# MarcioCerqueira/RealTimeDepthDiffusion

Measured on AMD Instinct MI355X. Metric: Mpixel-iterations/s (solver sweep), higher is better.
Workload: dtype f32

## Files before the change

realtimedepthdiffusion_amd/csrc/api.cpp:

```cpp
#include <climits>
#include <cmath>
#include <cstring>
#include <new>

#include "rtdd_internal.hpp"
#include "persist_sync.hpp"

namespace rtdd {

int fail(rtdd_ctx *ctx, int status, const char *what, hipError_t e) {
    if (ctx) {
        ctx->last_error = what ? what : "";
        if (e != hipSuccess) {
            ctx->last_error += ": ";
            ctx->last_error += hipGetErrorString(e);
        }
    }
    return status;
}

void omega_schedule(int n, std::vector<float> &out) {
    out.resize(n > 0 ? n : 0);
    const int S = 10;
    float omega = 0.0f;
    const float rho = 0.99;
    for (int it = 0; it < n; it++) {
        if (it < S) omega = 1;
        else if (it == S) omega = 2.0 / (2.0 - rho * rho);
        else omega = 4.0 / (4.0 - rho * rho * omega);
        out[it] = omega;
    }
}

static void free_levels(rtdd_ctx *ctx) {
    for (auto &L : ctx->levels) {
        for (auto &p : L.plane)
            if (p) { (void)hipFree(p); p = nullptr; }
        if (L.meta) { (void)hipFree(L.meta); L.meta = nullptr; }
    }
    ctx->levels.clear();
    ctx->maxLevel = -1;
}

}

using namespace rtdd;

#pragma GCC visibility push(default)
extern "C" {

int rtdd_version(void) { return RTDD_VERSION; }

const char *rtdd_status_string(int s) {
    switch (s) {
        case RTDD_OK: return "ok";
        case RTDD_ERR_INVALID: return "invalid argument";
        case RTDD_ERR_STATE: return "call order violated";
        case RTDD_ERR_HIP: return "HIP runtime error";
        case RTDD_ERR_NOMEM: return "out of memory";
        case RTDD_ERR_NO_DEVICE: return "no usable HIP device (there is no CPU fallback)";
        case RTDD_ERR_TIMEOUT: return "persistent kernel timed out (workgroups not co-resident)";
        default: return "unknown status";
    }
}

const char *rtdd_last_error(rtdd_ctx *ctx) { return ctx ? ctx->last_error.c_str() : "null context"; }

int rtdd_ctx_create(int device, rtdd_ctx **out) {
    if (!out) return RTDD_ERR_INVALID;
    *out = nullptr;
    int n = 0;
    if (hipGetDeviceCount(&n) != hipSuccess || n <= 0) return RTDD_ERR_NO_DEVICE;
    if (device < 0 || device >= n) return RTDD_ERR_INVALID;
    rtdd_ctx *ctx = new (std::nothrow) rtdd_ctx();
    if (!ctx) return RTDD_ERR_NOMEM;
    ctx->device = device;
    for (auto &t : ctx->persist_fit) t[0] = t[1] = -1;
    DeviceGuard g(device);
    hipDeviceProp_t prop;
    if (hipGetDeviceProperties(&prop, device) == hipSuccess) ctx->num_cus = prop.multiProcessorCount > 0 ? prop.multiProcessorCount : 256;
    bool ok = hipMalloc((void **)&ctx->lut_dev, 257 * sizeof(float)) == hipSuccess &&
              hipMalloc((void **)&ctx->residual_dev, 64) == hipSuccess &&
              hipMalloc((void **)&ctx->sync_words, kSyncWords * sizeof(int)) == hipSuccess &&
              hipMemset(ctx->sync_words, 0, kSyncWords * sizeof(int)) == hipSuccess;
    for (auto &e : ctx->ev) ok = ok && hipEventCreate(&e) == hipSuccess;
    if (ok && hipHostMalloc((void **)&ctx->confirm_host, 64, hipHostMallocMapped) == hipSuccess) {
        *ctx->confirm_host = 0;
        void *dev_view = nullptr;
        ok = hipHostGetDevicePointer(&dev_view, ctx->confirm_host, 0) == hipSuccess &&
             hipMemcpy(ctx->sync_words + kSyncConfirmPtr, &dev_view, sizeof(dev_view), hipMemcpyHostToDevice) == hipSuccess;
    } else ok = false;
    if (!ok) { rtdd_ctx_destroy(ctx); return RTDD_ERR_HIP; }
    *out = ctx;
    return RTDD_OK;
}

int rtdd_ctx_destroy(rtdd_ctx *ctx) {
    if (!ctx) return RTDD_OK;
    DeviceGuard g(ctx->device);
    (void)hipStreamSynchronize(ctx->stream);
    pyramid_free(ctx);
    mg_release(ctx);
    free_levels(ctx);
    if (ctx->lut_dev) (void)hipFree(ctx->lut_dev);
    if (ctx->omega_dev) (void)hipFree(ctx->omega_dev);
    if (ctx->residual_dev) (void)hipFree(ctx->residual_dev);
    if (ctx->sync_words) (void)hipFree(ctx->sync_words);
    if (ctx->sat) (void)hipFree(ctx->sat);
    if (ctx->bounce.ptr) (void)hipFree(ctx->bounce.ptr);
    if (ctx->confirm_host) (void)hipHostFree(ctx->confirm_host);
    for (auto &e : ctx->ev) if (e) (void)hipEventDestroy(e);
    delete ctx;
    return RTDD_OK;
}

int rtdd_ctx_set_stream(rtdd_ctx *ctx, rtdd_stream stream) {
    if (!ctx) return RTDD_ERR_INVALID;
    DeviceGuard g(ctx->device);
    RTDD_TRY(settle_pending(ctx));
    ctx->stream = (hipStream_t)stream;
    return RTDD_OK;
}

int rtdd_ctx_synchronize(rtdd_ctx *ctx) {
    if (!ctx) return RTDD_ERR_INVALID;
    DeviceGuard g(ctx->device);
    RTDD_HIP(ctx, hipStreamSynchronize(ctx->stream));
    return check_persistent_status(ctx);
}

static const struct OptionRow {
    int key;
    int Options::*member;
    bool zero_or_one;
    int lo, hi; const char *refusal;
} kOptions[] = {
    {RTDD_OPT_FP_CONTRACT, &Options::fp_contract, true, 0, 1, nullptr},
    {RTDD_OPT_SWEEP_KERNEL, &Options::sweep_kernel, false, 0, 2, "sweep kernel must be 0..2"},
    {RTDD_OPT_TEMPORAL_DEPTH, &Options::temporal_depth, false, 0, 28, "temporal depth must be 0..28"},
    {RTDD_OPT_ROWS_PER_WAVE, &Options::rows_per_wave, false, 0, 1024, "rows per wave must be 0..1024"},
    {RTDD_OPT_DEFOCUS_PATH, &Options::defocus_path, false, 0, 2, "defocus path must be 0..2"},
    {RTDD_OPT_TILE, &Options::tile, false, 0, 16, "tile must be 0..16"},
    {RTDD_OPT_PERSISTENT, &Options::persistent, true, 0, 1, nullptr},
    {RTDD_OPT_ANNOTATION_LDS, &Options::annotation_lds, true, 0, 1, nullptr},
    {RTDD_OPT_LIVE_ZERO_COPY, &Options::live_zero_copy, false, 0, 2, "RTDD_OPT_LIVE_ZERO_COPY is 0, 1 or 2"},
    {RTDD_OPT_TIMEOUT_HEAL, &Options::timeout_heal, true, 0, 1, nullptr},
    {RTDD_OPT_PERSISTENT_REARM_AFTER, &Options::rearm_after, false, 0, 1 << 20, "must be 0..2^20"},
    {RTDD_OPT_DEFOCUS_SLICE_MB, &Options::defocus_slice_mb, false, 0, 4095, "must be 0..4095 MB"},
    {RTDD_OPT_DEFOCUS_STRIPS, &Options::defocus_strips, false, 0, 2, "must be 0, 1 or 2"},
    {RTDD_OPT_AUTO_CYCLE_FIXED_NS, &Options::auto_cycle_fixed_ns, false, 0, INT_MAX, "must be >= 0"},
    {RTDD_OPT_AUTO_CYCLE_FS_PER_PX, &Options::auto_cycle_fs_per_px, false, 0, INT_MAX, "must be >= 0"},
    {RTDD_OPT_AUTO_SWEEP_FS_PER_PX, &Options::auto_sweep_fs_per_px, false, 0, INT_MAX, "must be >= 0"},
    {RTDD_OPT_AUTO_SWEEP_FLOOR_NS, &Options::auto_sweep_floor_ns, false, 0, INT_MAX, "must be >= 0"},
    {RTDD_OPT_DEBUG_WITHHOLD_TILE, &Options::debug_withhold_tile, false, 0, kSyncMaxTiles, "tile number + 1 out of range"},
    {RTDD_OPT_DEBUG_POLL_LIMIT_US, &Options::debug_poll_limit_us, false, 0, 10000000, "poll limit must be 0..1e7 us"},
    {RTDD_OPT_DEBUG_FORCE_STATUS, &Options::debug_force_status, false, 0, 3, "status must be 0..3"},
};
static const OptionRow *find_option(int key) {
    for (const OptionRow &r : kOptions) if (r.key == key) return &r;
    return nullptr;
}

int rtdd_set_option(rtdd_ctx *ctx, int key, int value) {
    if (!ctx) return RTDD_ERR_INVALID;
    const OptionRow *r = find_option(key);
    if (!r) return fail(ctx, RTDD_ERR_INVALID, "unknown option");
    if (r->zero_or_one) value = value ? 1 : 0;
    else REQUIRE(ctx, value >= r->lo && value <= r->hi, r->refusal);
    ctx->opt.*(r->member) = value;
    switch (key) {
        case RTDD_OPT_DEFOCUS_PATH: if (value == 0) ctx->defocus_table_sticky = ctx->defocus_band_sticky = false; break;
        case RTDD_OPT_PERSISTENT: ctx->persistent_wanted = value; ctx->persist_suspend = 0; break;
        case RTDD_OPT_TIMEOUT_HEAL: if (!value && !ctx->healing) { ctx->pending.clear(); ctx->pending_overflow = false; } break;
        default: break;
    }
    return RTDD_OK;
}

int rtdd_get_option(rtdd_ctx *ctx, int key, int *value) {
    if (!ctx || !value) return RTDD_ERR_INVALID;
    if (const OptionRow *r = find_option(key)) { *value = ctx->opt.*(r->member); return RTDD_OK; }
    switch (key) {
        case RTDD_OPT_TIMEOUT_HEALS: *value = ctx->heals; break;
        case RTDD_OPT_DEFOCUS_LAST_PATH: *value = ctx->defocus_last_path; break;
        case RTDD_OPT_DEFOCUS_LAST_SLICES: *value = ctx->defocus_last_slices; break;
        case RTDD_OPT_PERSISTENT_SUSPENDED: *value = ctx->persist_suspend; break;
        case RTDD_OPT_PENDING_CALLS: prune_confirmed(ctx); *value = (int)ctx->pending.size(); break;
        default: return fail(ctx, RTDD_ERR_INVALID, "unknown option");
    }
    return RTDD_OK;
}

int rtdd_profile_enable(rtdd_ctx *ctx, int on) {
    if (!ctx) return RTDD_ERR_INVALID;
    ctx->profile_on = on != 0;
    ctx->prof_pending = 0;
    return RTDD_OK;
}

int rtdd_profile_get(rtdd_ctx *ctx, rtdd_profile *out) {
    if (!ctx || !out) return RTDD_ERR_INVALID;
    DeviceGuard g(ctx->device);
    rtdd_profile p{};
    const int n = ctx->prof_pending < rtdd_ctx::kProfSlots ? ctx->prof_pending : rtdd_ctx::kProfSlots;
    for (int i = 0; i < n; i++) {
        const int slot = (ctx->prof_pending - 1 - i) % rtdd_ctx::kProfSlots;
        hipEvent_t *ev = ctx->ev + 4 * slot;
        RTDD_HIP(ctx, hipEventSynchronize(ev[3]));
        float a = 0, b = 0, c = 0;
        RTDD_HIP(ctx, hipEventElapsedTime(&a, ev[0], ev[1]));
        RTDD_HIP(ctx, hipEventElapsedTime(&b, ev[1], ev[2]));
        RTDD_HIP(ctx, hipEventElapsedTime(&c, ev[2], ev[3]));
        p.prepare_ms += a; p.sweep_ms += b; p.finish_ms += c;
        p.launches += ctx->prof_launches[slot]; p.sweeps += ctx->prof_sweeps[slot];
    }
    ctx->prof_pending = 0;
    ctx->prof = p;
    *out = p;
    return RTDD_OK;
}


int rtdd_allocate(rtdd_ctx *ctx, int rows, int cols, int levels) {
    if (!ctx) return RTDD_ERR_INVALID;
    REQUIRE(ctx, rows > 0 && cols > 0 && levels > 0 && levels <= 30, "rows, cols, levels must be positive");
    DeviceGuard g(ctx->device);
    RTDD_TRY(settle_pending(ctx));
    RTDD_HIP(ctx, hipStreamSynchronize(ctx->stream));
    free_levels(ctx);
    const int images = ctx->alloc_images > 0 ? ctx->alloc_images : 1;
    ctx->alloc_images = 1;
    ctx->levels.resize(levels);
    for (int l = 0; l < levels; l++) {
        Level &L = ctx->levels[l];
        L.rows = (int)(rows / powf(2, l));
        L.cols = (int)(cols / powf(2, l));
        L.elems = plane_elems(L.rows > 0 ? L.rows : 1, L.cols > 0 ? L.cols : 1);
        const size_t all = L.elems * (size_t)images;
        for (auto &p : L.plane) {
            hipError_t e = hipMalloc((void **)&p, all * sizeof(float));
            if (e != hipSuccess) { free_levels(ctx); return fail(ctx, e == hipErrorOutOfMemory ? RTDD_ERR_NOMEM : RTDD_ERR_HIP,
                "hipMalloc(plane)", e); }
        }
        hipError_t e = hipMalloc((void **)&L.meta, all * sizeof(uint32_t));
        if (e != hipSuccess) { free_levels(ctx); return fail(ctx, e == hipErrorOutOfMemory ? RTDD_ERR_NOMEM : RTDD_ERR_HIP,
            "hipMalloc(meta)", e); }
        for (auto &p : L.plane) RTDD_HIP(ctx, hipMemsetAsync(p, 0, all * sizeof(float), ctx->stream));
        RTDD_HIP(ctx, hipMemsetAsync(L.meta, 0, all * sizeof(uint32_t), ctx->stream));
    }
    ctx->levels_images = images;
    ctx->maxLevel = levels - 1;
    RTDD_HIP(ctx, hipStreamSynchronize(ctx->stream));
    return RTDD_OK;
}

int rtdd_free(rtdd_ctx *ctx) {
    if (!ctx) return RTDD_ERR_INVALID;
    DeviceGuard g(ctx->device);
    RTDD_TRY(settle_pending(ctx));
    RTDD_HIP(ctx, hipStreamSynchronize(ctx->stream));
    mg_release(ctx);
    free_levels(ctx);
    return RTDD_OK;
}

int rtdd_load_weights(rtdd_ctx *ctx, float beta) {
    if (!ctx) return RTDD_ERR_INVALID;
    DeviceGuard g(ctx->device);
    RTDD_TRY(settle_pending(ctx));
    for (int w = 0; w < 256; w++) ctx->lut_host[w] = expf(-beta * w);
    ctx->lut_host[256] = 0;
    RTDD_HIP(ctx, hipMemcpyAsync(ctx->lut_dev, ctx->lut_host, sizeof(ctx->lut_host), hipMemcpyHostToDevice, ctx->stream));
    RTDD_HIP(ctx, hipStreamSynchronize(ctx->stream));
    ctx->weights_loaded = true;
    return RTDD_OK;
}

static int ensure_omegas(rtdd_ctx *ctx, int n) {
    if (n <= ctx->omega_cap) return RTDD_OK;
    int cap = n < 1024 ? 1024 : n;
    std::vector<float> om;
    omega_schedule(cap, om);
    RTDD_HIP(ctx, hipStreamSynchronize(ctx->stream));
    if (ctx->omega_dev) { RTDD_HIP(ctx, hipFree(ctx->omega_dev)); ctx->omega_dev = nullptr; ctx->omega_cap = 0; }
    RTDD_HIP(ctx, hipMalloc((void **)&ctx->omega_dev, (size_t)cap * sizeof(float)));
    RTDD_HIP(ctx, hipMemcpy(ctx->omega_dev, om.data(), (size_t)cap * sizeof(float), hipMemcpyHostToDevice));
    ctx->omega_cap = cap;
    return RTDD_OK;
}

static constexpr int kAutoMaxCycles = 60;

static int check_solve_args(rtdd_ctx *ctx, const SolveCall &c) {
    REQUIRE(ctx, c.depth && c.scribble && c.gray, "null image pointer");
    REQUIRE(ctx, c.rows > 0 && c.cols > 0, "rows and cols must be positive");
    REQUIRE(ctx, f32_image_aligned(c.depth, c.depthPitch), kF32AlignText);
    REQUIRE(ctx, c.depthPitch >= (size_t)c.cols * sizeof(float), "depth pitch smaller than a row");
    REQUIRE(ctx, c.guide == RTDD_GUIDE_GRAY || c.guide == RTDD_GUIDE_BGR, "unknown guide kind");
    REQUIRE(ctx, c.scribblePitch >= (size_t)c.cols && c.grayPitch >= (size_t)c.cols * (c.guide == RTDD_GUIDE_BGR ? 3 : 1), "u8 pitch smaller than a row");
    REQUIRE(ctx, (c.regionFlags & ~(RTDD_REGION_CUT | RTDD_REGION_SMOOTH)) == 0, "unknown region flag");
    REQUIRE(ctx, c.regionFlags == 0 || (c.regions && c.regionsPitch >= (size_t)c.cols), "region flags without a region image, or its pitch smaller than a row");
    if (ctx->levels.empty()) return fail(ctx, RTDD_ERR_STATE, "rtdd_allocate has not been called");
    if (!ctx->weights_loaded) return fail(ctx, RTDD_ERR_STATE, "rtdd_load_weights has not been called");
    REQUIRE(ctx, c.level >= 0 && c.level < (int)ctx->levels.size(), "level out of range");
    const Level &L = ctx->levels[c.level];
    REQUIRE(ctx, plane_elems(c.rows, c.cols) <= L.elems, "rows x cols exceeds the level's allocation");
    return RTDD_OK;
}

namespace {

struct Solve {
    rtdd_ctx *ctx;
    const Level &L;
    size_t ip;
    int rows, cols;
    const rtdd_solve_params *p;
    int images;
    int done = 0, launches = 0, cycles = 0;
    int pk = 0, pm = 1;
    float residual = NAN;

    bool stop_on_residual() const { return p->tolerance > 0.0f; }
    bool reached() const { return residual <= p->tolerance; }
    int check() { return launch_residual(ctx, L, ip, pk, rows, cols, &residual); }

    int chebyshev_jacobi() {
        std::vector<float> omegas;
        omega_schedule(p->maxIterations, omegas);
        const bool blocked = ctx->opt.sweep_kernel != 1;
        const float *omegas_dev = nullptr;
        int rc;
        if (blocked && p->maxIterations > 0) {
            if ((rc = ensure_omegas(ctx, p->maxIterations)) != RTDD_OK) return rc;
            omegas_dev = ctx->omega_dev;
        }
        const int chunk = stop_on_residual() ? (p->checkEvery > 0 ? p->checkEvery : 16) : p->maxIterations;
        while (done < p->maxIterations) {
            const int n = p->maxIterations - done < chunk ? p->maxIterations - done : chunk;
            int ln = 0;
            rc = blocked ? launch_sweeps_blocked(ctx, L, ip, rows, cols, omegas_dev + done, n, &pk, &pm, &ln, images)
                         : launch_sweeps(ctx, L, ip, rows, cols, omegas.data() + done, n, &pk, &pm, &ln);
            if (rc != RTDD_OK) return rc;
            done += n; launches += ln;
            if (stop_on_residual()) {
                if ((rc = check()) != RTDD_OK) return rc;
                if (reached()) break;
            }
        }
        return RTDD_OK;
    }

    int red_black_sweeps(int n, float omega) {
        if (n > p->maxIterations - done) n = p->maxIterations - done;
        if (n <= 0) return RTDD_OK;
        int ln = 2 * n, rc;
        if (ctx->opt.sweep_kernel == 1) rc = launch_rbgs(ctx, L, ip, pk, rows, cols, n, omega);
        else rc = launch_rbgs_blocked(ctx, L, ip, rows, cols, n, omega, &pk, &ln);
        done += n; launches += ln;
        return rc;
    }

    int red_black() {
        const int chunk = stop_on_residual() ? (p->checkEvery > 0 ? p->checkEvery : 16) : (p->maxIterations > 0 ? p->maxIterations : 1);
        const float omega = p->relaxation == 0.0f ? 1.0f : p->relaxation;
        int rc;
        while (done < p->maxIterations) {
            if ((rc = red_black_sweeps(chunk, omega)) != RTDD_OK) return rc;
            if (stop_on_residual()) {
                if ((rc = check()) != RTDD_OK) return rc;
                if (reached()) break;
            }
        }
        return RTDD_OK;
    }

    int sor_cycles(bool after_vcycles) {
        const int longest = rows > cols ? rows : cols;
        const int base = after_vcycles ? (longest + 1) / 2 : longest;
        double w0 = 2.0 / (1.0 + sin(4.0 * 3.14159265358979323846 / (double)longest));
        if (w0 > 1.99) w0 = 1.99;
        if (w0 < 1.0) w0 = 1.0;
        bool ok = false;
        int rc;
        for (int cycle = 0; done < p->maxIterations && !ok; cycle++) {
            const int e = cycle < 6 ? cycle : 6;
            double gap = (2.0 - w0) / (double)(1 << e);
            if (gap < 0.005) gap = 0.005;
            const float w_hi = (float)(2.0 - gap);
            float w_mid = (float)(2.0 - 10.0 * gap);
            if (w_mid < 1.0f) w_mid = 1.0f;
            const int n_hi = base << e;
            if ((rc = red_black_sweeps(n_hi, w_hi)) != RTDD_OK) return rc;
            if ((rc = red_black_sweeps(n_hi / 4, w_mid)) != RTDD_OK) return rc;
            for (int k = 0; k < 5 && done < p->maxIterations && !ok; k++) {
                if ((rc = red_black_sweeps(20, 1.0f)) != RTDD_OK) return rc;
                if (stop_on_residual()) {
                    if ((rc = check()) != RTDD_OK) return rc;
                    ok = reached();
                }
            }
        }
        return RTDD_OK;
    }

    int vcycles(int max_cycles, int check_every, double alternative_seconds) {
        const double px = (double)rows * cols;
        const double cycle_seconds = ctx->opt.auto_cycle_fixed_ns * 1e-9 + px * ctx->opt.auto_cycle_fs_per_px * 1e-15;
        return launch_multigrid(ctx, L, ip, rows, cols, max_cycles, p->tolerance, check_every, alternative_seconds, cycle_seconds, &pk,
            &cycles, &residual, &launches);
    }

    int automatic() {
        const int longest = rows > cols ? rows : cols;
        const double px = (double)rows * cols;
        const double per_px = px * ctx->opt.auto_sweep_fs_per_px * 1e-15, floor_s = ctx->opt.auto_sweep_floor_ns * 1e-9;
        const double sweep_seconds = per_px > floor_s ? per_px : floor_s;
        const double sor_seconds = ((double)((longest + 1) / 2) * 1.25 + 20.0) * sweep_seconds;
        const int rc = vcycles(kAutoMaxCycles, 1, sor_seconds);
        if (rc != RTDD_OK || reached()) return rc;
        return sor_cycles(true);
    }
};

}

static int solve_once(rtdd_ctx *ctx, const SolveCall &c, int seq, SolveOutcome *out) {
    const SolveTargets &t = c.targets;
    const Level L = ctx->levels[c.level].view(t.batch.first);
    const size_t ip = plane_pitch(c.cols);
    const bool prof = ctx->profile_on;
    hipEvent_t *ev = ctx->ev + 4 * (ctx->prof_pending % rtdd_ctx::kProfSlots);

    if (prof) RTDD_HIP(ctx, hipEventRecord(ev[0], ctx->stream));
    ctx->wild_seq = seq;
    int rc = launch_prepare(ctx, L, ip, c);
    if (rc != RTDD_OK) return rc;
    if (prof) RTDD_HIP(ctx, hipEventRecord(ev[1], ctx->stream));

    ctx->last_info = rtdd_solve_info{};
    ctx->last_info.residual = NAN;
    Solve s{ctx, L, ip, c.rows, c.cols, &c.params, t.batch.n};
    switch (c.params.method) {
        case RTDD_METHOD_CHEBYSHEV_JACOBI: rc = s.chebyshev_jacobi(); break;
        case RTDD_METHOD_MULTIGRID:
            rc = s.vcycles(c.params.maxIterations, c.params.checkEvery > 0 ? c.params.checkEvery : 1, 0.0);
            s.done = s.cycles;
            break;
        case RTDD_METHOD_AUTO: rc = s.automatic(); break;
        default: rc = c.params.relaxation < 0.0f ? s.sor_cycles(false) : s.red_black(); break;
    }
    if (rc != RTDD_OK) return rc;

    if (prof) RTDD_HIP(ctx, hipEventRecord(ev[2], ctx->stream));
    if (out) { out->plane = s.pk; out->seq = seq; }
    if (!t.defer_finish) {
        rc = launch_finish(ctx, L, ip, s.pk, c, seq);
        if (rc != RTDD_OK) return rc;
    }
    if (prof) {
        RTDD_HIP(ctx, hipEventRecord(ev[3], ctx->stream));
        const int slot = ctx->prof_pending % rtdd_ctx::kProfSlots;
        ctx->prof_launches[slot] = s.launches; ctx->prof_sweeps[slot] = s.done;
        ctx->prof_pending++;
    }
    ctx->last_info.iterations = s.done; ctx->last_info.residual = s.residual; ctx->last_info.cycles = s.cycles;
    ctx->last_info.fp_contract = ctx->opt.fp_contract; ctx->last_info.launches = s.launches;
    return RTDD_OK;
}

int rtdd_solve_ex(rtdd_ctx *ctx, float *depth, size_t depthPitch, const uint8_t *scribble, size_t scribblePitch,
                  const uint8_t *gray, size_t grayPitch, int rows, int cols, int level,
                  const rtdd_solve_params *params, rtdd_solve_info *info) {
    if (!ctx) return RTDD_ERR_INVALID;
    REQUIRE(ctx, params != nullptr, "null params");
    return solve_with(ctx, {depth, depthPitch, scribble, scribblePitch, gray, grayPitch, RTDD_GUIDE_GRAY, rows, cols, level, *params, {}}, info, nullptr);
}

int rtdd_solve_guided(rtdd_ctx *ctx, float *depth, size_t depthPitch, const uint8_t *scribble, size_t scribblePitch,
                      const uint8_t *guide, size_t guidePitch, int guideKind, int rows, int cols, int level,
                      const rtdd_solve_params *params, rtdd_solve_info *info) {
    if (!ctx) return RTDD_ERR_INVALID;
    REQUIRE(ctx, params != nullptr, "null params");
    return solve_with(ctx, {depth, depthPitch, scribble, scribblePitch, guide, guidePitch, guideKind, rows, cols, level, *params, {}}, info, nullptr);
}

int rtdd_solve_regions(rtdd_ctx *ctx, float *depth, size_t depthPitch, const uint8_t *scribble, size_t scribblePitch,
                       const uint8_t *guide, size_t guidePitch, int guideKind, const uint8_t *regions, size_t regionsPitch, int regionFlags,
                       int rows, int cols, int level, const rtdd_solve_params *params, rtdd_solve_info *info) {
    if (!ctx) return RTDD_ERR_INVALID;
    REQUIRE(ctx, params != nullptr, "null params");
    REQUIRE(ctx, (regionFlags & ~(RTDD_REGION_CUT | RTDD_REGION_SMOOTH)) == 0, "unknown region flag");
    REQUIRE(ctx, regions || regionFlags == 0, "region flags without a region image");
    REQUIRE(ctx, !regions || cols <= 0 || regionsPitch >= (size_t)cols, "region pitch smaller than a row");
    SolveCall c{depth, depthPitch, scribble, scribblePitch, guide, guidePitch, guideKind, rows, cols, level, *params, {}};
    if (regions && regionFlags != 0) { c.regions = regions; c.regionsPitch = regionsPitch; c.regionFlags = regionFlags; }
    return solve_with(ctx, c, info, nullptr);
}

}
#pragma GCC visibility pop

int rtdd::solve_with(rtdd_ctx *ctx, const SolveCall &c, rtdd_solve_info *info, SolveOutcome *out) {
    if (!ctx) return RTDD_ERR_INVALID;
    const SolveTargets &t = c.targets;
    REQUIRE(ctx, c.params.maxIterations >= 0, "maxIterations must be >= 0");
    REQUIRE(ctx, c.params.method == RTDD_METHOD_CHEBYSHEV_JACOBI || c.params.method == RTDD_METHOD_RED_BLACK_GS ||
                 c.params.method == RTDD_METHOD_MULTIGRID || c.params.method == RTDD_METHOD_AUTO, "unknown method");
    REQUIRE(ctx, c.params.method != RTDD_METHOD_AUTO || c.params.tolerance > 0.0f, "RTDD_METHOD_AUTO needs a tolerance");
    REQUIRE(ctx, c.params.method != RTDD_METHOD_RED_BLACK_GS || c.params.relaxation == RTDD_RELAXATION_AUTO ||
                 (c.params.relaxation >= 0.0f && c.params.relaxation < 2.0f), "relaxation must be in [0,2) or RTDD_RELAXATION_AUTO");
    RTDD_TRY(check_solve_args(ctx, c));
    REQUIRE(ctx, t.batch.first >= 0 && t.batch.n >= 1 && t.batch.first + t.batch.n <= ctx->levels_images,
            "the batch exceeds what the context's levels were allocated for");
    REQUIRE(ctx, t.batch.n == 1 || (c.params.method == RTDD_METHOD_CHEBYSHEV_JACOBI && c.params.tolerance <= 0.0f && ctx->opt.sweep_kernel != 1),
            "a batched solve runs the reference's scheme with the temporally blocked kernel only");
    DeviceGuard g(ctx->device);
    if (ctx->solve_seq >= (1 << 30)) {
        if (!ctx->healing) RTDD_TRY(settle_pending(ctx));
        RTDD_HIP(ctx, hipStreamSynchronize(ctx->stream));
        *(volatile int *)ctx->confirm_host = 0;
        RTDD_HIP(ctx, hipMemset(ctx->sync_words + kSyncWild, 0, sizeof(int)));
        ctx->solve_seq = 0; ctx->publish_seq = 0;
    }
    const int seq = ++ctx->solve_seq;
    const Options asked = ctx->opt;
    int rc = solve_once(ctx, c, seq, out);
    if (rc == kRestartSolve) rc = solve_once(ctx, c, seq, out);
    if (rc == kRestartSolve) rc = fail(ctx, RTDD_ERR_TIMEOUT, "the solve was restarted after a timed-out persistent launch and failed again");
    if (rc != RTDD_OK) return rc;
    if (!ctx->healing && ctx->persist_suspend > 0 && --ctx->persist_suspend == 0 && ctx->persistent_wanted) ctx->opt.persistent = 1;
    if (t.logged) {
        PendingOp op;
        op.kind = PendingOp::kSolve; op.opt = asked; op.solve = c; op.seq = seq;
        log_call(ctx, op);
    }
    if (info) *info = ctx->last_info;
    return RTDD_OK;
}

#pragma GCC visibility push(default)
extern "C" {

int rtdd_last_solve_info(rtdd_ctx *ctx, rtdd_solve_info *info) {
    if (!ctx || !info) return RTDD_ERR_INVALID;
    *info = ctx->last_info;
    return RTDD_OK;
}

int rtdd_multigrid_level(rtdd_ctx *ctx, int level, int which, float *host, int *rows, int *cols) {
    if (!ctx) return RTDD_ERR_INVALID;
    REQUIRE(ctx, rows && cols, "null size pointers");
    DeviceGuard g(ctx->device);
    const int rc = mg_download(ctx, level, which, host, rows, cols);
    if (rc == RTDD_ERR_INVALID) return fail(ctx, rc, "no multigrid hierarchy, or level/plane out of range");
    return rc;
}

int rtdd_matrix_free_solver(rtdd_ctx *ctx, float *depth, size_t depthPitch, const uint8_t *scribble, size_t scribblePitch,
                            const uint8_t *gray, size_t grayPitch, int rows, int cols, float beta, int maxIterations,
                            float tolerance, int level) {
    (void)beta; (void)tolerance;
    if (!ctx) return RTDD_ERR_INVALID;
    if (maxIterations < 0) maxIterations = 0;
    const rtdd_solve_params p{RTDD_METHOD_CHEBYSHEV_JACOBI, maxIterations, 0.0f, 0, 0.0f};
    return solve_with(ctx, {depth, depthPitch, scribble, scribblePitch, gray, grayPitch, RTDD_GUIDE_GRAY, rows, cols, level, p, {}}, nullptr, nullptr);
}

int rtdd_index_to_weight(rtdd_ctx *ctx, const uint8_t *gray, size_t grayPitch, const float *depth, size_t depthPitch,
                         int32_t *index2, int level, int rows, int cols) {
    return rtdd_index_to_weight_guided(ctx, gray, grayPitch, RTDD_GUIDE_GRAY, depth, depthPitch, index2, level, rows, cols);
}

int rtdd_index_to_weight_guided(rtdd_ctx *ctx, const uint8_t *guide, size_t guidePitch, int guideKind, const float *depth, size_t depthPitch,
                                int32_t *index2, int level, int rows, int cols) {
    return rtdd_index_to_weight_regions(ctx, guide, guidePitch, guideKind, nullptr, 0, 0, depth, depthPitch, index2, level, rows, cols);
}

int rtdd_index_to_weight_regions(rtdd_ctx *ctx, const uint8_t *guide, size_t guidePitch, int guideKind, const uint8_t *regions, size_t regionsPitch,
                                 int regionFlags, const float *depth, size_t depthPitch, int32_t *index2, int level, int rows, int cols) {
    if (!ctx) return RTDD_ERR_INVALID;
    REQUIRE(ctx, (regionFlags & ~(RTDD_REGION_CUT | RTDD_REGION_SMOOTH)) == 0, "unknown region flag");
    REQUIRE(ctx, regions || regionFlags == 0, "region flags without a region image");
    REQUIRE(ctx, !regions || cols <= 0 || regionsPitch >= (size_t)cols, "region pitch smaller than a row");
    if (!regions) regionFlags = 0;
    const uint8_t *gray = guide;
    REQUIRE(ctx, guideKind == RTDD_GUIDE_GRAY || guideKind == RTDD_GUIDE_BGR, "unknown guide kind");
    const size_t grayPitch = guideKind == RTDD_GUIDE_BGR ? guidePitch / 3 : guidePitch;
    REQUIRE(ctx, gray && depth && index2, "null pointer");
    REQUIRE(ctx, rows > 0 && cols > 0 && grayPitch >= (size_t)cols && depthPitch >= (size_t)cols * 4, "bad size or pitch");
    REQUIRE(ctx, f32_image_aligned(depth, depthPitch), kF32AlignText);
    if (ctx->maxLevel < 0) return fail(ctx, RTDD_ERR_STATE, "rtdd_allocate has not been called (maxLevel unknown)");
    DeviceGuard g(ctx->device);
    RTDD_TRY(settle_pending(ctx));
    return launch_index_to_weight(ctx, guide, guidePitch, depth, depthPitch, index2, level, rows, cols, guideKind, regions, regionsPitch, regionFlags);
}

int rtdd_region_codes(rtdd_ctx *ctx, const uint8_t *edited, size_t editedPitch, const uint8_t *mask, size_t maskPitch, int rows, int cols,
                      int level, uint8_t *codes, size_t codesPitch) {
    if (!ctx) return RTDD_ERR_INVALID;
    REQUIRE(ctx, edited && mask && codes, "null image pointer");
    REQUIRE(ctx, rows >= 0 && cols >= 0 && rows <= 32768 && cols <= 32768, "size outside [0, 32768]");
    REQUIRE(ctx, level >= 0 && level < 16, "level outside [0, 15]");
    RegionLevels lv{};
    lv.n = 1; lv.shift[0] = level; lv.rows[0] = rows >> level; lv.cols[0] = cols >> level;
    if (lv.rows[0] == 0 || lv.cols[0] == 0) return RTDD_OK;
    REQUIRE(ctx, editedPitch >= (size_t)cols * 3 && maskPitch >= (size_t)cols && codesPitch >= (size_t)lv.cols[0], "pitch smaller than a row");
    lv.codes[0] = codes; lv.pitch[0] = codesPitch; lv.stride[0] = 0;
    DeviceGuard g(ctx->device);
    RTDD_TRY(pyramid_check_read(ctx, mask, edited));
    return launch_region_codes(ctx, edited, editedPitch, 0, mask, maskPitch, 0, lv, 1);
}

}
#pragma GCC visibility pop
```

realtimedepthdiffusion_amd/csrc/rtdd_internal.hpp:

```cpp
#pragma once

#include <hip/hip_runtime.h>

#include <cmath>
#include <cstdint>
#include <cstdio>
#include <string>
#include <vector>

#include "rtdd.h"

namespace rtdd {

constexpr int kGuardRows = 16;
constexpr int kGuardCols = 64;
constexpr int kRowAlign = 64;

inline size_t plane_pitch(int cols) { return (size_t)((cols + kRowAlign - 1) / kRowAlign) * kRowAlign + kGuardCols; }
inline size_t plane_elems(int rows, int cols) { return plane_pitch(cols) * (size_t)(rows + 2 * kGuardRows) + 1024; }

constexpr uint32_t kMetaDirichlet = 1u << 16;

struct Level {
    int rows = 0, cols = 0;
    size_t elems = 0;
    float *plane[4] = {nullptr, nullptr, nullptr, nullptr};
    uint32_t *meta = nullptr;
    float *P(int i, size_t ip) const { return plane[i] + (size_t)kGuardRows * ip; }
    uint32_t *M(size_t ip) const { return meta + (size_t)kGuardRows * ip; }
    Level view(int b) const {
        Level v = *this;
        for (auto &q : v.plane) if (q) q += (size_t)b * elems;
        if (v.meta) v.meta += (size_t)b * elems;
        return v;
    }
};

struct Batch {
    int n = 1;
    int first = 0;
    size_t depth = 0, scribble = 0, gray = 0, u8 = 0;
    size_t regions = 0;
};
#define RTDD_Z(ptr, stride) ptr = (decltype(ptr))((const char *)(ptr) + (size_t)blockIdx.z * (size_t)(stride))

struct SolveTargets {
    Batch batch;
    bool defer_finish = false;
    uint8_t *u8 = nullptr; size_t u8_pitch = 0;
    uint8_t *u8b = nullptr; size_t u8b_pitch = 0;
    bool logged = true;
};
struct SolveOutcome { int seq = 0, plane = -1; };
struct SolveCall {
    float *depth = nullptr; size_t depthPitch = 0;
    const uint8_t *scribble = nullptr; size_t scribblePitch = 0;
    const uint8_t *gray = nullptr; size_t grayPitch = 0;
    int guide = RTDD_GUIDE_GRAY;
    int rows = 0, cols = 0, level = 0;
    rtdd_solve_params params{};
    SolveTargets targets;
    const uint8_t *regions = nullptr; size_t regionsPitch = 0;
    int regionFlags = 0;
};
struct LiveTargets {
    void *scribble = nullptr, *edited = nullptr;
    uint8_t *u8 = nullptr; size_t u8_pitch = 0;
    int effect = 0;
    uint8_t *artistic = nullptr; size_t artistic_pitch = 0;
};

struct Effect {
    enum : int { kRefocus = RTDD_EFFECT_HAZE + 1, kHazeEx, kStereo, kLensBlur, kRelight, kRelightShadow, kParallax, kAmbientOcclusion, kLighting, kBokeh, kComposite, kRemove, kLift, kParallaxLayered };
    int kind = RTDD_EFFECT_NONE;
    const uint8_t *original = nullptr; size_t originalPitch = 0;
    const float *depth = nullptr; size_t depthPitch = 0;
    uint8_t *artistic = nullptr; size_t artisticPitch = 0;
    int rows = 0, cols = 0;
    const uint8_t *gray = nullptr; size_t grayPitch = 0;
    int kernelSize = 0, focusX = -1, focusY = -1;
    float focusDepth = 0.0f;
    float beta = 2.0f; uint32_t air = 0xFFFFFFu;
    int disparity = 0, zeroX = -1, zeroY = -1, stereoMode = 0;
    float zeroDepth = 0.0f;
    struct Light {
        int kind = 0, anchorX = -1, anchorY = -1;
        float x = 0.0f, y = 0.0f, z = 1.0f;
        float anchorDepth = 0.0f, invR2 = 0.0f;
        float relief = 0.0f, ambient = 0.0f, k[3] = {0.0f, 0.0f, 0.0f};
    } light = {};
    struct Shadow {
        float sx = 0.0f, sy = 0.0f, rise = 0.0f;
        int maxSteps = 0;
        float bias = 0.0f, softness = 0.0f, strength = 0.0f;
    } shadow = {};
    struct Parallax {
        int shiftX = 0, shiftY = 0, zeroX = -1, zeroY = -1;
        float dolly = 0.0f, zeroDepth = 0.0f;
        float cx = 0.0f, cy = 0.0f;
    } parallax = {};
    struct ParallaxLayers {
        const uint8_t *plate = nullptr; size_t platePitch = 0;
        const float *plateDepth = nullptr; size_t plateDepthPitch = 0;
        float *depthOut = nullptr; size_t depthOutPitch = 0;
        uint8_t *coverage = nullptr; size_t coveragePitch = 0;
    } layers = {};
    struct Occlusion {
        int mode = 0, directions = 8, radius = 0;
        float relief = 0.0f, bias = 0.0f, strength = 0.0f;
        bool lit = false;
    } occlusion = {};
    struct Composite {
        rtdd_layer layer = {};
        const uint8_t *sprite = nullptr; size_t spritePitch = 0;
        float *depthOut = nullptr; size_t depthOutPitch = 0;
        int fx0 = 0, fy0 = 0, fx1 = 0, fy1 = 0;
    } composite = {};
    struct Remove {
        rtdd_removal removal = {};
        const uint8_t *mask = nullptr; size_t maskPitch = 0;
        float *depthOut = nullptr; size_t depthOutPitch = 0;
    } remove = {};
    struct Lift {
        const uint8_t *mask = nullptr; size_t maskPitch = 0;
        int select = 0, x = 0, y = 0;
        uint8_t *sprite = nullptr; size_t spritePitch = 0;
        int spriteRows = 0, spriteCols = 0;
    } lift = {};
};

inline int window_scale(double aperture, int rows, int cols) {
    const double k = aperture * sqrtf(rows * rows + cols * cols);
    return k < 2147483647.0 ? (int)k : 2147483647;
}

struct Options {
    int fp_contract = 1;
    int sweep_kernel = 0;
    int temporal_depth = 0;
    int rows_per_wave = 0;
    int tile = 0;
    int persistent = 1;
    int defocus_path = 0;
    int auto_cycle_fixed_ns = 270000;
    int auto_cycle_fs_per_px = 46000;
    int auto_sweep_fs_per_px = 1429;
    int auto_sweep_floor_ns = 2500;
    int debug_withhold_tile = 0;
    int debug_poll_limit_us = 0;
    int debug_force_status = 0;
    int timeout_heal = 1;
    int annotation_lds = 1;
    int live_zero_copy = 1;
    int defocus_slice_mb = 0;
    int defocus_strips = 0;
    int rearm_after = 64;
};

struct PendingOp {
    enum Kind { kSolve = 0, kEstimate = 1, kEffect = 2 } kind = kSolve;
    Options opt;
    unsigned long long id = 0;
    SolveCall solve;
    int seq = 0;
    struct Estimate {
        int maxIterations = 0;
        int level_seq[32] = {};
        int batch_first = 0, batch_n = 1;
        int guide = RTDD_GUIDE_GRAY;
        int regionFlags = 0;
        LiveTargets live;
        int annotation = 0;
    } estimate;
    enum : int { kAnnotationNone = 0, kAnnotationAccumulated = 1, kAnnotationRebuilt = 2 };
    Effect effect;
};
constexpr int kRestartSolve = -1000;
constexpr size_t kMaxPendingOps = 4096;
constexpr int kMaxRearms = 4;

}

namespace rtdd { struct Pyramid; struct MgState; }

namespace rtdd {
struct Bounce { void *ptr = nullptr; size_t bytes = 0; };
}

struct rtdd_ctx {
    int device = 0;
    rtdd::Pyramid *pyr = nullptr;
    rtdd::MgState *mg = nullptr;
    hipStream_t stream = nullptr;
    std::vector<rtdd::Level> levels;
    int alloc_images = 1;
    int levels_images = 1;
    int maxLevel = -1;
    bool weights_loaded = false;
    float lut_host[257];
    float *lut_dev = nullptr;
    float *omega_dev = nullptr;
    int omega_cap = 0;
    float *residual_dev = nullptr;
    int *sync_words = nullptr;
    int defocus_last_path = 0;
    int defocus_last_slices = 0;
    bool defocus_band_sticky = false;
    bool defocus_table_sticky = false;
    int flag_epoch = 0;
    int sync_limit = 0;
    int last_nominal_depth = 0;
    int last_launch_images = 1;
    rtdd_solve_info last_info{};
    int solve_seq = 0;
    int wild_seq = -1;
    std::vector<rtdd::PendingOp> pending;
    bool pending_overflow = false;
    bool healing = false;
    bool heal_rebuilt = false;
    bool heal_warned = false;
    int heals = 0;
    int persistent_wanted = 1;
    int persist_suspend = 0;
    int *confirm_host = nullptr;
    unsigned long long op_counter = 0;
    bool persistent_used = false;
    int publish_seq = 0;
    bool status_writer_behind = false;
    signed char persist_fit[17][2];
    rtdd::Bounce bounce;
    uint32_t *sat = nullptr;
    size_t sat_elems = 0;
    int sat_rows = 0, sat_cols = 0;
    int num_cus = 256;
    rtdd::Options opt;
    bool profile_on = false;
    rtdd_profile prof{};
    static constexpr int kProfSlots = 64;
    hipEvent_t ev[4 * kProfSlots] = {};
    int prof_launches[kProfSlots] = {}, prof_sweeps[kProfSlots] = {};
    int prof_pending = 0;
    std::string last_error;
};

namespace rtdd {

#ifdef __HIPCC__
__device__ __forceinline__ int wave_id() { return __builtin_amdgcn_readfirstlane((int)(threadIdx.x >> 6)); }
#endif

int fail(rtdd_ctx *ctx, int status, const char *what, hipError_t e = hipSuccess);
inline bool f32_image_aligned(const void *p, size_t pitch) { return (uintptr_t)p % sizeof(float) == 0 && pitch % sizeof(float) == 0; }
constexpr const char *kF32AlignText = "an f32 image needs a pointer and a pitch that are multiples of 4";
inline void note_status_writer(rtdd_ctx *ctx) { ctx->persistent_used = true; ctx->status_writer_behind = true; }
inline void note_publisher(rtdd_ctx *ctx, int seq) { ctx->persistent_used = true; ctx->publish_seq = seq; ctx->status_writer_behind = false; }

#define RTDD_HIP(ctx, call)                                                        \
    do {                                                                           \
        hipError_t e_ = (call);                                                    \
        if (e_ != hipSuccess) return ::rtdd::fail((ctx), RTDD_ERR_HIP, #call, e_); \
    } while (0)

#define REQUIRE(ctx, cond, msg) \
    do { if (!(cond)) return ::rtdd::fail((ctx), RTDD_ERR_INVALID, msg); } while (0)
#define REQUIRE_PYRAMID(ctx)                                                                                             \
    do {                                                                                                                 \
        if (!(ctx)) return RTDD_ERR_INVALID;                                                                             \
        if (!(ctx)->pyr) return ::rtdd::fail((ctx), RTDD_ERR_STATE, "rtdd_pyramid_create has not been called");          \
    } while (0)
#define RTDD_TRY(call) \
    do { const int rc_ = (call); if (rc_ != RTDD_OK) return rc_; } while (0)

#define RTDD_LAUNCH_CHECK(ctx, name)                                                     \
    do {                                                                                 \
        hipError_t e_ = hipGetLastError();                                               \
        if (e_ != hipSuccess) return ::rtdd::fail((ctx), RTDD_ERR_HIP, "launch " name, e_); \
    } while (0)

struct DeviceGuard {
    int prev = -1;
    explicit DeviceGuard(int dev) {
        if (hipGetDevice(&prev) != hipSuccess) prev = -1;
        if (prev != dev) (void)hipSetDevice(dev);
        else prev = -1;
    }
    ~DeviceGuard() {
        if (prev >= 0) (void)hipSetDevice(prev);
    }
};

int launch_prepare(rtdd_ctx *ctx, const Level &L, size_t ip, const SolveCall &c);
int launch_sweeps(rtdd_ctx *ctx, const Level &L, size_t ip, int rows, int cols, const float *omegas_host, int n,
                  int *pk, int *pm, int *launches);
int launch_sweeps_blocked(rtdd_ctx *ctx, const Level &L, size_t ip, int rows, int cols, const float *omegas_dev, int n,
                          int *pk, int *pm, int *launches, int images = 1);
int launch_finish(rtdd_ctx *ctx, const Level &L, size_t ip, int src_plane, const SolveCall &c, int seq);
int launch_index_to_weight(rtdd_ctx *ctx, const uint8_t *gray, size_t grayPitch, const float *depth, size_t depthPitch,
                           int32_t *index2, int level, int rows, int cols, int guide = RTDD_GUIDE_GRAY,
                           const uint8_t *regions = nullptr, size_t regionsPitch = 0, int regionFlags = 0);
int launch_residual(rtdd_ctx *ctx, const Level &L, size_t ip, int plane, int rows, int cols, float *host_out);
int launch_rbgs(rtdd_ctx *ctx, const Level &L, size_t ip, int plane, int rows, int cols, int nsweeps, float omega);
int launch_multigrid(rtdd_ctx *ctx, const Level &L0, size_t ip, int rows, int cols, int max_cycles, float tolerance, int check_every, double alternative_seconds,
                     double cycle_seconds, int *plane, int *cycles_done, float *residual, int *launches);
void mg_release(rtdd_ctx *ctx);
int mg_download(rtdd_ctx *ctx, int level, int which, float *host, int *rows, int *cols);

int launch_rbgs_blocked(rtdd_ctx *ctx, const Level &L, size_t ip, int rows, int cols, int n, float omega, int *plane, int *launches, int keep = -1);

int launch_convert(rtdd_ctx *ctx, const uint8_t *src, size_t srcPitch, float *dst, size_t dstPitch,
                   const uint8_t *mask, size_t maskPitch, int rows, int cols, int images = 1, size_t zSrc = 0, size_t zDst = 0, size_t zMask = 0);
int launch_pyrdown_annotation(rtdd_ctx *ctx, const uint8_t *ps, size_t psp, const uint8_t *pe, size_t pep, int prows, int pcols,
                              uint8_t *cs, size_t csp, uint8_t *ce, size_t cep, int crows, int ccols,
                              int images = 1, size_t zPs = 0, size_t zPe = 0, size_t zCs = 0, size_t zCe = 0);
int launch_annotation_pyramid(rtdd_ctx *ctx, int levels, uint8_t *const *scribble, const size_t *sp, const size_t *zs, uint8_t *const *edited, const size_t *ep, const size_t *ze,
                              const int *rows, const int *cols, float *depth, size_t dp, size_t zd, int images, bool rebuild = false);
int launch_repitch(rtdd_ctx *ctx, hipStream_t stream, const void *src, size_t srcPitch, void *dst, size_t dstPitch, size_t widthBytes, int rows);
inline bool slow_pitch(size_t hostPitch, int rows) { return hostPitch % 4 != 0 && rows > 1; }
inline bool wants_bounce(size_t hostPitch, size_t widthBytes, int rows) { return slow_pitch(hostPitch, rows) && hostPitch == widthBytes; }
int copy_h2d_linear(rtdd_ctx *ctx, Bounce &b, void *dev, size_t devPitch, const void *host, size_t hostPitch, size_t widthBytes, int rows,
                    hipStream_t copyStream, hipStream_t kernelStream);
int copy_h2d_repitch(rtdd_ctx *ctx, const Bounce &b, void *dev, size_t devPitch, size_t hostPitch, size_t widthBytes, int rows, hipStream_t kernelStream);
int copy_h2d(rtdd_ctx *ctx, Bounce &b, void *dev, size_t devPitch, const void *host, size_t hostPitch, size_t widthBytes, int rows, hipStream_t stream);
int copy_d2h(rtdd_ctx *ctx, Bounce &b, void *host, size_t hostPitch, const void *dev, size_t devPitch, size_t widthBytes, int rows, hipStream_t stream);
struct PaintTarget {
    uint8_t *edited; size_t editedPitch;
    uint8_t *scribble; size_t scribblePitch;
    const uint8_t *original; size_t originalPitch;
    int rows, cols;
};
int launch_paint(rtdd_ctx *ctx, int x, int y, int color, int radius, const PaintTarget &t);
template <class Stroke> int launch_paint_strokes(rtdd_ctx *ctx, const Stroke *strokes, int count, const PaintTarget &t);

int launch_fill_polygon(rtdd_ctx *ctx, const int *xy, int n, const rtdd_fill &fill, const PaintTarget &t);

int launch_fill_similar(rtdd_ctx *ctx, const rtdd_wand &wand, const PaintTarget &t, rtdd_wand_info *info);
int launch_fill_surface(rtdd_ctx *ctx, const rtdd_surface_wand &wand, const PaintTarget &t, const float *depth, size_t depthPitch, rtdd_wand_info *info);

int launch_segment_surfaces(rtdd_ctx *ctx, const rtdd_segmentation &sg, const PaintTarget &t, const float *depth, size_t depthPitch, int32_t *labels,
                            size_t labelsPitch, rtdd_segment *segments, rtdd_segment_info *info);

int launch_effect(rtdd_ctx *ctx, const Effect &e);
int launch_lens_blur(rtdd_ctx *ctx, const Effect &e);
int launch_relight(rtdd_ctx *ctx, const Effect &e);
int launch_relight_shadow(rtdd_ctx *ctx, const Effect &e);
int launch_parallax(rtdd_ctx *ctx, const Effect &e);
int launch_ambient_occlusion(rtdd_ctx *ctx, const Effect &e);
int launch_lighting(rtdd_ctx *ctx, const Effect &e);
int launch_bokeh(rtdd_ctx *ctx, const Effect &e);
int launch_composite(rtdd_ctx *ctx, const Effect &e);
constexpr int kRemoveTile = 64, kRemoveGroup = 3, kRemoveApex = 8192, kRemoveApexChain = kRemoveApex + kRemoveApex / 2 + 64;
int launch_remove(rtdd_ctx *ctx, const Effect &e);
int launch_lift(rtdd_ctx *ctx, const Effect &e);

int launch_bgr2gray(rtdd_ctx *ctx, const uint8_t *bgr, size_t bp, uint8_t *gray, size_t gp, int rows, int cols);
int launch_pyrdown_u8(rtdd_ctx *ctx, const uint8_t *src, size_t sp, int rows, int cols, uint8_t *dst, size_t dp);
int launch_pyrdown_bgr(rtdd_ctx *ctx, const uint8_t *src, size_t sp, int rows, int cols, uint8_t *dst, size_t dp);
struct PyrupBatch { int n = 1; size_t src = 0, dst = 0, edited = 0, mask = 0, coarse = 0; };
int launch_pyrup_inject(rtdd_ctx *ctx, const float *src, size_t sp, int rows, int cols, float *dst, size_t dp, int drows, int dcols,
                        const uint8_t *edited, size_t ep, const uint8_t *mask, size_t mp, float *coarse_out = nullptr, size_t cp = 0,
                        int guard_seq = 0 , const PyrupBatch *batch = nullptr);
int launch_depth_to_u8(rtdd_ctx *ctx, const float *src, size_t sp, uint8_t *dst, size_t dp, int rows, int cols);
int launch_decode_annotation(rtdd_ctx *ctx, const uint8_t *bgr, size_t bp, const uint8_t *ann, size_t ap, uint8_t *edited, size_t ep,
                             uint8_t *scribble, size_t sp, int rows, int cols);
int launch_fill_f32(rtdd_ctx *ctx, float *dst, size_t dp, int rows, int cols, float v);
struct RegionLevels {
    static constexpr int kMax = 12;
    int n = 0;
    uint8_t *codes[kMax]; size_t pitch[kMax], stride[kMax];
    int rows[kMax], cols[kMax], shift[kMax], first_block[kMax + 1];
};
int launch_region_codes(rtdd_ctx *ctx, const uint8_t *edited, size_t ep, size_t ze, const uint8_t *mask, size_t mp, size_t zm, RegionLevels &lv, int images);
void pyramid_free(rtdd_ctx *ctx);
int pyramid_note_write(rtdd_ctx *ctx, const void *scribble, const void *edited, bool erases = false);
int pyramid_check_read(rtdd_ctx *ctx, const void *a, const void *b);

int prepare_persistent_launch(rtdd_ctx *ctx, int nblocks, int *flag_base);
int check_persistent_status(rtdd_ctx *ctx, bool in_solve = false);
void prune_confirmed(rtdd_ctx *ctx);
int settle_pending(rtdd_ctx *ctx);
bool log_call(rtdd_ctx *ctx, PendingOp &op);
int solve_with(rtdd_ctx *ctx, const SolveCall &c, rtdd_solve_info *info, SolveOutcome *out);
int estimate_replay(rtdd_ctx *ctx, const PendingOp::Estimate &e, int failed_seq);

void omega_schedule(int n, std::vector<float> &out);

}
```

realtimedepthdiffusion_amd/csrc/solver_kernels.hip:

```cpp
#include "rtdd_internal.hpp"
#include "persist_sync.hpp"

namespace rtdd {

__device__ __forceinline__ int sat_u8_dev(float v) {
    if (!(v >= 0.0f)) return 0;
    if (v >= 255.0f) return 255;
    return (int)v;
}

__device__ __forceinline__ int iabs(int a) { return a < 0 ? -a : a; }

__device__ __forceinline__ int region_index(int i, int rp, int rq, int flags) {
    if ((flags & RTDD_REGION_CUT) && rp != rq) return 255;
    if ((flags & RTDD_REGION_SMOOTH) && rp == rq && rp != 0) return 0;
    return i;
}
#define RTDD_PREPARE_PARAMS(g, gp, zg)                                                                                                      \
    const float *__restrict__ depth, size_t depthPitch, const uint8_t *__restrict__ scribble, size_t scribblePitch,                         \
    const uint8_t *__restrict__ g, size_t gp, float *__restrict__ X0, float *__restrict__ X1, uint32_t *__restrict__ M, int ip, int rows,    \
    int cols, int gated, int thr, size_t zDepth, size_t zScribble, size_t zg, size_t zPlane, int *sync_words, int wild_seq
#define RTDD_PREPARE_ARGS(g, gp, zg) \
    depth, depthPitch, scribble, scribblePitch, g, gp, X0, X1, M, ip, rows, cols, gated, thr, zDepth, zScribble, zg, zPlane, sync_words, wild_seq
#define RTDD_REGION_PARAMS const uint8_t *__restrict__ codes, size_t codesPitch, size_t zCodes, int regionFlags
#define RTDD_REGION_ARGS codes, codesPitch, zCodes, regionFlags
#define RTDD_NO_REGIONS nullptr, 0, 0, 0

template <bool REGIONS>
__device__ __forceinline__ void prepare_px(RTDD_PREPARE_PARAMS(gray, grayPitch, zGray), RTDD_REGION_PARAMS) {
    const int x = blockIdx.x * 64 + (threadIdx.x & 63);
    const int y = blockIdx.y * 4 + wave_id();
    if (x >= cols || y >= rows) return;
    RTDD_Z(depth, zDepth); RTDD_Z(scribble, zScribble); RTDD_Z(gray, zGray); RTDD_Z(X0, zPlane); RTDD_Z(X1, zPlane); RTDD_Z(M, zPlane);
    const float *drow = (const float *)((const char *)depth + (size_t)y * depthPitch);
    const uint8_t *grow = gray + (size_t)y * grayPitch;
    const float d = drow[x];
    const int g = grow[x];
    const bool dirichlet = scribble[(size_t)y * scribblePitch + x] == 255;
    const uint8_t *rrow = nullptr;
    if (REGIONS) { RTDD_Z(codes, zCodes); rrow = codes + (size_t)y * codesPitch; }
    int right = 0, down = 0;
    if (x + 1 < cols) {
        right = iabs(g - (int)grow[x + 1]);
        if (gated && !(iabs(sat_u8_dev(d) - sat_u8_dev(drow[x + 1])) > thr)) right = 0;
        if (REGIONS) right = region_index(right, rrow[x], rrow[x + 1], regionFlags);
    }
    if (y + 1 < rows) {
        down = iabs(g - (int)grow[x + grayPitch]);
        if (gated) {
            const float dd = ((const float *)((const char *)depth + (size_t)(y + 1) * depthPitch))[x];
            if (!(iabs(sat_u8_dev(d) - sat_u8_dev(dd)) > thr)) down = 0;
        }
        if (REGIONS) down = region_index(down, rrow[x], rrow[x + codesPitch], regionFlags);
    }
    const size_t p = (size_t)y * ip + x;
    if (depth_is_wild(d)) sync_words[kSyncWild] = wild_seq;
    X0[p] = d;
    X1[p] = dirichlet ? d : 0.0f;
    M[p] = (uint32_t)right | ((uint32_t)down << 8) | (dirichlet ? kMetaDirichlet : 0u);
}
__global__ __launch_bounds__(256) void k_prepare(RTDD_PREPARE_PARAMS(gray, grayPitch, zGray)) {
    prepare_px<false>(RTDD_PREPARE_ARGS(gray, grayPitch, zGray), RTDD_NO_REGIONS);
}
__global__ __launch_bounds__(256) void k_prepare_regions(RTDD_PREPARE_PARAMS(gray, grayPitch, zGray), RTDD_REGION_PARAMS) {
    prepare_px<true>(RTDD_PREPARE_ARGS(gray, grayPitch, zGray), RTDD_REGION_ARGS);
}

struct RegionCodes4 { int rc[5], rd[4]; };
template <bool REGIONS>
__device__ __forceinline__ void load_codes4(RegionCodes4 &r, const uint8_t *rrow, size_t codesPitch, int x0, int cols, bool down_ok) {
    if (!REGIONS) return;
    if (x0 + 3 < cols) {
        const uint32_t c4 = *(const uint32_t *)(rrow + x0);
        r.rc[0] = c4 & 255; r.rc[1] = (c4 >> 8) & 255; r.rc[2] = (c4 >> 16) & 255; r.rc[3] = c4 >> 24;
        if (down_ok) {
            const uint32_t e4 = *(const uint32_t *)(rrow + codesPitch + x0);
            r.rd[0] = e4 & 255; r.rd[1] = (e4 >> 8) & 255; r.rd[2] = (e4 >> 16) & 255; r.rd[3] = e4 >> 24;
        }
    } else {
#pragma unroll
        for (int i = 0; i < 4; i++) {
            const bool in = x0 + i < cols;
            r.rc[i] = in ? rrow[x0 + i] : 0;
            r.rd[i] = in && down_ok ? rrow[x0 + i + codesPitch] : 0;
        }
    }
    r.rc[4] = x0 + 4 < cols ? rrow[x0 + 4] : 0;
}

template <bool REGIONS>
__device__ __forceinline__ void prepare4_px(RTDD_PREPARE_PARAMS(gray, grayPitch, zGray), RTDD_REGION_PARAMS) {
    const int x0 = 4 * (blockIdx.x * 64 + (threadIdx.x & 63));
    const int y = blockIdx.y * 4 + wave_id();
    if (x0 >= cols || y >= rows) return;
    RTDD_Z(depth, zDepth); RTDD_Z(scribble, zScribble); RTDD_Z(gray, zGray); RTDD_Z(X0, zPlane); RTDD_Z(X1, zPlane); RTDD_Z(M, zPlane);
    const float *drow = (const float *)((const char *)depth + (size_t)y * depthPitch);
    const uint8_t *grow = gray + (size_t)y * grayPitch, *srow = scribble + (size_t)y * scribblePitch;
    const bool down_ok = y + 1 < rows;
    float d[5], dd[4];
    int g[5], gd[4];
    uint32_t sc;
    RegionCodes4 rg;
    if (REGIONS) { RTDD_Z(codes, zCodes); load_codes4<REGIONS>(rg, codes + (size_t)y * codesPitch, codesPitch, x0, cols, down_ok); }
    if (x0 + 3 < cols) {
        const float4 d4 = *(const float4 *)(drow + x0);
        d[0] = d4.x; d[1] = d4.y; d[2] = d4.z; d[3] = d4.w;
        const uint32_t g4 = *(const uint32_t *)(grow + x0);
        g[0] = g4 & 255; g[1] = (g4 >> 8) & 255; g[2] = (g4 >> 16) & 255; g[3] = g4 >> 24;
        sc = *(const uint32_t *)(srow + x0);
        if (down_ok) {
            const uint32_t h4 = *(const uint32_t *)(grow + grayPitch + x0);
            gd[0] = h4 & 255; gd[1] = (h4 >> 8) & 255; gd[2] = (h4 >> 16) & 255; gd[3] = h4 >> 24;
            if (gated) { const float4 e4 = *(const float4 *)((const float *)((const char *)depth + (size_t)(y + 1) * depthPitch) + x0); dd[0] = e4.x; dd[1] = e4.y; dd[2] = e4.z; dd[3] = e4.w; }
        }
    } else {
        sc = 0;
#pragma unroll
        for (int i = 0; i < 4; i++) {
            const bool in = x0 + i < cols;
            d[i] = in ? drow[x0 + i] : 0.0f; g[i] = in ? grow[x0 + i] : 0;
            sc |= (uint32_t)(in ? srow[x0 + i] : 0) << (8 * i);
            gd[i] = in && down_ok ? grow[x0 + i + grayPitch] : 0;
            dd[i] = in && down_ok && gated ? ((const float *)((const char *)depth + (size_t)(y + 1) * depthPitch))[x0 + i] : 0.0f;
        }
    }
    const bool right_ok = x0 + 4 < cols;
    d[4] = right_ok ? drow[x0 + 4] : 0.0f; g[4] = right_ok ? grow[x0 + 4] : 0;
    float x0v[4], x1v[4];
    uint32_t mv[4];
#pragma unroll
    for (int i = 0; i < 4; i++) {
        const bool dirichlet = ((sc >> (8 * i)) & 255) == 255;
        int right = 0, down = 0;
        if (x0 + i + 1 < cols) {
            right = iabs(g[i] - g[i + 1]);
            if (gated && !(iabs(sat_u8_dev(d[i]) - sat_u8_dev(d[i + 1])) > thr)) right = 0;
            if (REGIONS) right = region_index(right, rg.rc[i], rg.rc[i + 1], regionFlags);
        }
        if (down_ok) {
            down = iabs(g[i] - gd[i]);
            if (gated && !(iabs(sat_u8_dev(d[i]) - sat_u8_dev(dd[i])) > thr)) down = 0;
            if (REGIONS) down = region_index(down, rg.rc[i], rg.rd[i], regionFlags);
        }
        x0v[i] = d[i];
        x1v[i] = dirichlet ? d[i] : 0.0f;
        mv[i] = (uint32_t)right | ((uint32_t)down << 8) | (dirichlet ? kMetaDirichlet : 0u);
    }
    if (depth_is_wild(d[0]) || depth_is_wild(d[1]) || depth_is_wild(d[2]) || depth_is_wild(d[3])) sync_words[kSyncWild] = wild_seq;
    const size_t p = (size_t)y * ip + x0;
    *(float4 *)(X0 + p) = make_float4(x0v[0], x0v[1], x0v[2], x0v[3]);
    *(float4 *)(X1 + p) = make_float4(x1v[0], x1v[1], x1v[2], x1v[3]);
    *(uint4 *)(M + p) = make_uint4(mv[0], mv[1], mv[2], mv[3]);
}
__global__ __launch_bounds__(256) void k_prepare4(RTDD_PREPARE_PARAMS(gray, grayPitch, zGray)) {
    prepare4_px<false>(RTDD_PREPARE_ARGS(gray, grayPitch, zGray), RTDD_NO_REGIONS);
}
__global__ __launch_bounds__(256) void k_prepare4_regions(RTDD_PREPARE_PARAMS(gray, grayPitch, zGray), RTDD_REGION_PARAMS) {
    prepare4_px<true>(RTDD_PREPARE_ARGS(gray, grayPitch, zGray), RTDD_REGION_ARGS);
}

template <bool REGIONS> struct RegionImage {};
template <> struct RegionImage<true> { const uint8_t *codes; size_t pitch; int flags; };
__device__ __forceinline__ int region_index(int i, int x, int y, int nx, int ny, const RegionImage<true> &rg) {
    return region_index(i, rg.codes[(size_t)y * rg.pitch + x], rg.codes[(size_t)ny * rg.pitch + nx], rg.flags);
}
__device__ __forceinline__ int region_index(int i, int, int, int, int, const RegionImage<false> &) { return i; }

template <bool REGIONS>
__global__ __launch_bounds__(256) void k_index_to_weight(const uint8_t *__restrict__ gray, size_t grayPitch,
                                                         const float *__restrict__ depth, size_t depthPitch,
                                                         int32_t *__restrict__ index2, int rows, int cols, int gated, int thr, const RegionImage<REGIONS> rg) {
    const int x = blockIdx.x * 64 + (threadIdx.x & 63);
    const int y = blockIdx.y * 4 + wave_id();
    if (x >= cols || y >= rows) return;
    const int g = gray[(size_t)y * grayPitch + x];
    const float *drow = (const float *)((const char *)depth + (size_t)y * depthPitch);
    const int d = gated ? sat_u8_dev(drow[x]) : 0;
    int idx[4] = {256, 256, 256, 256};
    const int dx[4] = {-1, 1, 0, 0}, dy[4] = {0, 0, -1, 1};
#pragma unroll
    for (int k = 0; k < 4; k++) {
        const int nx = x + dx[k], ny = y + dy[k];
        if (nx < 0 || ny < 0 || nx >= cols || ny >= rows) continue;
        int v = iabs(g - (int)gray[(size_t)ny * grayPitch + nx]);
        if (gated) {
            const float nd = ((const float *)((const char *)depth + (size_t)ny * depthPitch))[nx];
            if (!(iabs(d - sat_u8_dev(nd)) > thr)) v = 0;
        }
        if (REGIONS) v = region_index(v, x, y, nx, ny, rg);
        idx[k] = v;
    }
    const size_t p = (size_t)y * cols + x;
    index2[2 * p + 0] = idx[0] * 1000 + idx[1];
    index2[2 * p + 1] = idx[2] * 1000 + idx[3];
}

__device__ __forceinline__ int bgr_at(const uint8_t *p) { return (int)p[0] | ((int)p[1] << 8) | ((int)p[2] << 16); }
__device__ __forceinline__ int bgr_index(int p, int q) {
    const int db = iabs((p & 255) - (q & 255)), dg = iabs(((p >> 8) & 255) - ((q >> 8) & 255)), dr = iabs((p >> 16) - (q >> 16));
    return max(max(db, dg), dr);
}

template <bool REGIONS>
__device__ __forceinline__ void prepare_bgr_px(RTDD_PREPARE_PARAMS(bgr, bgrPitch, zBgr), RTDD_REGION_PARAMS) {
    const int x = blockIdx.x * 64 + (threadIdx.x & 63);
    const int y = blockIdx.y * 4 + wave_id();
    if (x >= cols || y >= rows) return;
    RTDD_Z(depth, zDepth); RTDD_Z(scribble, zScribble); RTDD_Z(bgr, zBgr); RTDD_Z(X0, zPlane); RTDD_Z(X1, zPlane); RTDD_Z(M, zPlane);
    const float *drow = (const float *)((const char *)depth + (size_t)y * depthPitch);
    const uint8_t *crow = bgr + (size_t)y * bgrPitch + 3 * (size_t)x;
    const float d = drow[x];
    const int c = bgr_at(crow);
    const bool dirichlet = scribble[(size_t)y * scribblePitch + x] == 255;
    const uint8_t *rrow = nullptr;
    if (REGIONS) { RTDD_Z(codes, zCodes); rrow = codes + (size_t)y * codesPitch; }
    int right = 0, down = 0;
    if (x + 1 < cols) {
        right = bgr_index(c, bgr_at(crow + 3));
        if (gated && !(iabs(sat_u8_dev(d) - sat_u8_dev(drow[x + 1])) > thr)) right = 0;
        if (REGIONS) right = region_index(right, rrow[x], rrow[x + 1], regionFlags);
    }
    if (y + 1 < rows) {
        down = bgr_index(c, bgr_at(crow + bgrPitch));
        if (gated) {
            const float dd = ((const float *)((const char *)depth + (size_t)(y + 1) * depthPitch))[x];
            if (!(iabs(sat_u8_dev(d) - sat_u8_dev(dd)) > thr)) down = 0;
        }
        if (REGIONS) down = region_index(down, rrow[x], rrow[x + codesPitch], regionFlags);
    }
    const size_t p = (size_t)y * ip + x;
    if (depth_is_wild(d)) sync_words[kSyncWild] = wild_seq;
    X0[p] = d;
    X1[p] = dirichlet ? d : 0.0f;
    M[p] = (uint32_t)right | ((uint32_t)down << 8) | (dirichlet ? kMetaDirichlet : 0u);
}
__global__ __launch_bounds__(256) void k_prepare_bgr(RTDD_PREPARE_PARAMS(bgr, bgrPitch, zBgr)) {
    prepare_bgr_px<false>(RTDD_PREPARE_ARGS(bgr, bgrPitch, zBgr), RTDD_NO_REGIONS);
}
__global__ __launch_bounds__(256) void k_prepare_bgr_regions(RTDD_PREPARE_PARAMS(bgr, bgrPitch, zBgr), RTDD_REGION_PARAMS) {
    prepare_bgr_px<true>(RTDD_PREPARE_ARGS(bgr, bgrPitch, zBgr), RTDD_REGION_ARGS);
}

__device__ __forceinline__ void bgr_unpack4(const uint8_t *q, int (&c)[5]) {
    const uint32_t *w = (const uint32_t *)q;
    const uint32_t w0 = w[0], w1 = w[1], w2 = w[2];
    c[0] = (int)(w0 & 0xFFFFFFu); c[1] = (int)((w0 >> 24) | ((w1 & 0xFFFFu) << 8));
    c[2] = (int)((w1 >> 16) | ((w2 & 0xFFu) << 16)); c[3] = (int)(w2 >> 8);
}

template <bool REGIONS>
__device__ __forceinline__ void prepare4_bgr_px(RTDD_PREPARE_PARAMS(bgr, bgrPitch, zBgr), RTDD_REGION_PARAMS) {
    const int x0 = 4 * (blockIdx.x * 64 + (threadIdx.x & 63));
    const int y = blockIdx.y * 4 + wave_id();
    if (x0 >= cols || y >= rows) return;
    RTDD_Z(depth, zDepth); RTDD_Z(scribble, zScribble); RTDD_Z(bgr, zBgr); RTDD_Z(X0, zPlane); RTDD_Z(X1, zPlane); RTDD_Z(M, zPlane);
    const float *drow = (const float *)((const char *)depth + (size_t)y * depthPitch);
    const uint8_t *crow = bgr + (size_t)y * bgrPitch + 3 * (size_t)x0, *srow = scribble + (size_t)y * scribblePitch;
    const bool down_ok = y + 1 < rows;
    float d[5], dd[4];
    int c[5], cd[5];
    uint32_t sc;
    RegionCodes4 rg;
    if (REGIONS) { RTDD_Z(codes, zCodes); load_codes4<REGIONS>(rg, codes + (size_t)y * codesPitch, codesPitch, x0, cols, down_ok); }
    if (x0 + 3 < cols) {
        const float4 d4 = *(const float4 *)(drow + x0);
        d[0] = d4.x; d[1] = d4.y; d[2] = d4.z; d[3] = d4.w;
        bgr_unpack4(crow, c);
        sc = *(const uint32_t *)(srow + x0);
        if (down_ok) {
            bgr_unpack4(crow + bgrPitch, cd);
            if (gated) { const float4 e4 = *(const float4 *)((const float *)((const char *)depth + (size_t)(y + 1) * depthPitch) + x0); dd[0] = e4.x; dd[1] = e4.y; dd[2] = e4.z; dd[3] = e4.w; }
        }
    } else {
        sc = 0;
#pragma unroll
        for (int i = 0; i < 4; i++) {
            const bool in = x0 + i < cols;
            d[i] = in ? drow[x0 + i] : 0.0f; c[i] = in ? bgr_at(crow + 3 * i) : 0;
            sc |= (uint32_t)(in ? srow[x0 + i] : 0) << (8 * i);
            cd[i] = in && down_ok ? bgr_at(crow + bgrPitch + 3 * i) : 0;
            dd[i] = in && down_ok && gated ? ((const float *)((const char *)depth + (size_t)(y + 1) * depthPitch))[x0 + i] : 0.0f;
        }
    }
    const bool right_ok = x0 + 4 < cols;
    d[4] = right_ok ? drow[x0 + 4] : 0.0f;
    c[4] = right_ok ? (int)*(const uint16_t *)(crow + 12) | ((int)crow[14] << 16) : 0;
    float x0v[4], x1v[4];
    uint32_t mv[4];
#pragma unroll
    for (int i = 0; i < 4; i++) {
        const bool dirichlet = ((sc >> (8 * i)) & 255) == 255;
        int right = 0, down = 0;
        if (x0 + i + 1 < cols) {
            right = bgr_index(c[i], c[i + 1]);
            if (gated && !(iabs(sat_u8_dev(d[i]) - sat_u8_dev(d[i + 1])) > thr)) right = 0;
            if (REGIONS) right = region_index(right, rg.rc[i], rg.rc[i + 1], regionFlags);
        }
        if (down_ok) {
            down = bgr_index(c[i], cd[i]);
            if (gated && !(iabs(sat_u8_dev(d[i]) - sat_u8_dev(dd[i])) > thr)) down = 0;
            if (REGIONS) down = region_index(down, rg.rc[i], rg.rd[i], regionFlags);
        }
        x0v[i] = d[i];
        x1v[i] = dirichlet ? d[i] : 0.0f;
        mv[i] = (uint32_t)right | ((uint32_t)down << 8) | (dirichlet ? kMetaDirichlet : 0u);
    }
    if (depth_is_wild(d[0]) || depth_is_wild(d[1]) || depth_is_wild(d[2]) || depth_is_wild(d[3])) sync_words[kSyncWild] = wild_seq;
    const size_t p = (size_t)y * ip + x0;
    *(float4 *)(X0 + p) = make_float4(x0v[0], x0v[1], x0v[2], x0v[3]);
    *(float4 *)(X1 + p) = make_float4(x1v[0], x1v[1], x1v[2], x1v[3]);
    *(uint4 *)(M + p) = make_uint4(mv[0], mv[1], mv[2], mv[3]);
}
__global__ __launch_bounds__(256) void k_prepare4_bgr(RTDD_PREPARE_PARAMS(bgr, bgrPitch, zBgr)) {
    prepare4_bgr_px<false>(RTDD_PREPARE_ARGS(bgr, bgrPitch, zBgr), RTDD_NO_REGIONS);
}
__global__ __launch_bounds__(256) void k_prepare4_bgr_regions(RTDD_PREPARE_PARAMS(bgr, bgrPitch, zBgr), RTDD_REGION_PARAMS) {
    prepare4_bgr_px<true>(RTDD_PREPARE_ARGS(bgr, bgrPitch, zBgr), RTDD_REGION_ARGS);
}

template <bool REGIONS>
__global__ __launch_bounds__(256) void k_index_to_weight_bgr(const uint8_t *__restrict__ bgr, size_t bgrPitch,
                                                             const float *__restrict__ depth, size_t depthPitch,
                                                             int32_t *__restrict__ index2, int rows, int cols, int gated, int thr, const RegionImage<REGIONS> rg) {
    const int x = blockIdx.x * 64 + (threadIdx.x & 63);
    const int y = blockIdx.y * 4 + wave_id();
    if (x >= cols || y >= rows) return;
    const int c = bgr_at(bgr + (size_t)y * bgrPitch + 3 * (size_t)x);
    const float *drow = (const float *)((const char *)depth + (size_t)y * depthPitch);
    const int d = gated ? sat_u8_dev(drow[x]) : 0;
    int idx[4] = {256, 256, 256, 256};
    const int dx[4] = {-1, 1, 0, 0}, dy[4] = {0, 0, -1, 1};
#pragma unroll
    for (int k = 0; k < 4; k++) {
        const int nx = x + dx[k], ny = y + dy[k];
        if (nx < 0 || ny < 0 || nx >= cols || ny >= rows) continue;
        int v = bgr_index(c, bgr_at(bgr + (size_t)ny * bgrPitch + 3 * (size_t)nx));
        if (gated) {
            const float nd = ((const float *)((const char *)depth + (size_t)ny * depthPitch))[nx];
            if (!(iabs(d - sat_u8_dev(nd)) > thr)) v = 0;
        }
        if (REGIONS) v = region_index(v, x, y, nx, ny, rg);
        idx[k] = v;
    }
    const size_t p = (size_t)y * cols + x;
    index2[2 * p + 0] = idx[0] * 1000 + idx[1];
    index2[2 * p + 1] = idx[2] * 1000 + idx[3];
}

template <bool CONTRACT>
__device__ __forceinline__ float mean4(float xl, float xr, float xu, float xd, float wl, float wr, float wu, float wd,
                                       bool vl, bool vr, bool vu, bool vd) {
    float sum = 0.0f, cnt = 0.0f, s2;
    s2 = CONTRACT ? __builtin_fmaf(wl, xl, sum) : sum + wl * xl;  sum = vl ? s2 : sum;  cnt = vl ? cnt + wl : cnt;
    s2 = CONTRACT ? __builtin_fmaf(wr, xr, sum) : sum + wr * xr;  sum = vr ? s2 : sum;  cnt = vr ? cnt + wr : cnt;
    s2 = CONTRACT ? __builtin_fmaf(wu, xu, sum) : sum + wu * xu;  sum = vu ? s2 : sum;  cnt = vu ? cnt + wu : cnt;
    s2 = CONTRACT ? __builtin_fmaf(wd, xd, sum) : sum + wd * xd;  sum = vd ? s2 : sum;  cnt = vd ? cnt + wd : cnt;
    float r = sum / cnt;
    if (!(r >= 0.0f)) r = 0.0f;
    if (r > 255.0f) r = 255.0f;
    if (cnt == 0.0f) r = 0.0f;
    return r;
}

template <bool CONTRACT>
__device__ __forceinline__ float chebyshev(float r, float x, float prev, float omega, float gamma) {
    if (CONTRACT) return __builtin_fmaf(omega, __builtin_fmaf(gamma, r - x, x) - prev, prev);
    return (omega * (gamma * (r - x) + x - prev)) + prev;
}

template <bool CONTRACT>
__global__ __launch_bounds__(256) void k_sweep1(const float *__restrict__ X, float *__restrict__ Y,
                                                const uint32_t *__restrict__ M, const float *__restrict__ lut_g,
                                                int ip, int rows, int cols, int R, float omega, float gamma) {
    __shared__ float lut[257];
    for (int i = threadIdx.x; i < 257; i += 256) lut[i] = lut_g[i];
    __syncthreads();

    const int lane = threadIdx.x & 63;
    const int wave = wave_id();
    const int x0 = blockIdx.x * 256 + lane * 4;
    const int ybeg = (blockIdx.y * 4 + wave) * R;
    const int yend = min(ybeg + R, rows);
    if (ybeg >= rows) return;

    const bool lane_in = x0 < cols;
    const bool vl0 = x0 > 0;
    bool vr[4];
#pragma unroll
    for (int i = 0; i < 4; i++) vr[i] = x0 + i + 1 < cols;

    const float *xrow = X + (size_t)ybeg * ip + x0;
    float4 up = *(const float4 *)(xrow - ip);
    float4 cur = *(const float4 *)(xrow);
    float wu[4];
    {
        const uint4 mu = *(const uint4 *)(M + (size_t)(ybeg - 1) * ip + x0);
        wu[0] = lut[(mu.x >> 8) & 255]; wu[1] = lut[(mu.y >> 8) & 255];
        wu[2] = lut[(mu.z >> 8) & 255]; wu[3] = lut[(mu.w >> 8) & 255];
    }

    for (int y = ybeg; y < yend; y++) {
        const size_t rowoff = (size_t)y * ip + x0;
        const float4 dn = *(const float4 *)(X + rowoff + ip);
        const uint4 m = *(const uint4 *)(M + rowoff);
        const float4 pv = *(const float4 *)(Y + rowoff);

        float xl = __shfl_up(cur.w, 1);
        float xr = __shfl_down(cur.x, 1);
        uint32_t ml = __shfl_up(m.w, 1);
        if (lane == 0) { xl = X[rowoff - 1]; ml = M[rowoff - 1]; }
        if (lane == 63) xr = X[rowoff + 4];

        const float wr[4] = {lut[m.x & 255], lut[m.y & 255], lut[m.z & 255], lut[m.w & 255]};
        const float wd[4] = {lut[(m.x >> 8) & 255], lut[(m.y >> 8) & 255], lut[(m.z >> 8) & 255], lut[(m.w >> 8) & 255]};
        const float wl0 = lut[ml & 255];
        const bool vu = y > 0, vd = y + 1 < rows;

        const float xc[4] = {cur.x, cur.y, cur.z, cur.w};
        const float xu[4] = {up.x, up.y, up.z, up.w};
        const float xd[4] = {dn.x, dn.y, dn.z, dn.w};
        const float pp[4] = {pv.x, pv.y, pv.z, pv.w};
        const uint32_t mm[4] = {m.x, m.y, m.z, m.w};
        float o[4];
#pragma unroll
        for (int i = 0; i < 4; i++) {
            const float r = mean4<CONTRACT>(i == 0 ? xl : xc[i - 1], i == 3 ? xr : xc[i + 1], xu[i], xd[i],
                                            i == 0 ? wl0 : wr[i - 1], wr[i], wu[i], wd[i],
                                            i == 0 ? vl0 : true, vr[i], vu, vd);
            const float v = chebyshev<CONTRACT>(r, xc[i], pp[i], omega, gamma);
            o[i] = (mm[i] & kMetaDirichlet) ? xc[i] : v;
        }
        if (lane_in) *(float4 *)(Y + rowoff) = make_float4(o[0], o[1], o[2], o[3]);
        up = cur; cur = dn;
#pragma unroll
        for (int i = 0; i < 4; i++) wu[i] = wd[i];
    }
}

__device__ __forceinline__ uint8_t round_u8(float v) {
    const float r = __builtin_rintf(v);
    return !(r >= 0.0f) ? 0 : (r >= 255.0f ? 255 : (uint8_t)(int)r);
}

__global__ __launch_bounds__(256) void k_finish(const float *__restrict__ X, int ip, float *__restrict__ depth, size_t depthPitch,
                                                int rows, int cols, uint8_t *__restrict__ u8, size_t u8Pitch, int *sync_words, int seq,
                                                size_t zPlane, size_t zDepth, size_t zU8, uint8_t *__restrict__ u8b, size_t u8bPitch) {
    const int x = blockIdx.x * 64 + (threadIdx.x & 63);
    const int y = blockIdx.y * 4 + wave_id();
    if (solve_is_dead(sync_words, seq, (blockIdx.x | blockIdx.y | blockIdx.z | threadIdx.x) == 0)) return;
    if (x >= cols || y >= rows) return;
    RTDD_Z(X, zPlane); RTDD_Z(depth, zDepth); if (u8) RTDD_Z(u8, zU8);
    const float v = X[(size_t)y * ip + x];
    ((float *)((char *)depth + (size_t)y * depthPitch))[x] = v;
    if (u8) u8[(size_t)y * u8Pitch + x] = round_u8(v);
    if (u8b) u8b[(size_t)y * u8bPitch + x] = round_u8(v);
}

__global__ __launch_bounds__(256) void k_finish4(const float *__restrict__ X, int ip, float *__restrict__ depth, size_t depthPitch,
                                                 int rows, int cols, uint8_t *__restrict__ u8, size_t u8Pitch, int *sync_words, int seq,
                                                 size_t zPlane, size_t zDepth, size_t zU8, uint8_t *__restrict__ u8b, size_t u8bPitch) {
    const int x0 = 4 * (blockIdx.x * 64 + (threadIdx.x & 63));
    const int y = blockIdx.y * 4 + wave_id();
    if (solve_is_dead(sync_words, seq, (blockIdx.x | blockIdx.y | blockIdx.z | threadIdx.x) == 0)) return;
    if (x0 >= cols || y >= rows) return;
    RTDD_Z(X, zPlane); RTDD_Z(depth, zDepth); if (u8) RTDD_Z(u8, zU8);
    const float4 v = *(const float4 *)(X + (size_t)y * ip + x0);
    float *o = (float *)((char *)depth + (size_t)y * depthPitch) + x0;
    const float t[4] = {v.x, v.y, v.z, v.w};
    if (x0 + 3 < cols) *(float4 *)o = v;
    else { for (int i = 0; i < 4; i++) if (x0 + i < cols) o[i] = t[i]; }
    uint8_t *targets[2] = {u8, u8b};
    const size_t pitches[2] = {u8Pitch, u8bPitch};
#pragma unroll
    for (int k = 0; k < 2; k++) {
        if (!targets[k]) continue;
        uint8_t *q = targets[k] + (size_t)y * pitches[k] + x0;
        if (x0 + 3 < cols && pitches[k] % 4 == 0 && (uintptr_t)targets[k] % 4 == 0)
            *(uint32_t *)q = (uint32_t)round_u8(t[0]) | ((uint32_t)round_u8(t[1]) << 8) | ((uint32_t)round_u8(t[2]) << 16) | ((uint32_t)round_u8(t[3]) << 24);
        else { for (int i = 0; i < 4; i++) if (x0 + i < cols) q[i] = round_u8(t[i]); }
    }
}

template <bool CONTRACT>
__device__ __forceinline__ float mean_at(const float *__restrict__ X, const uint32_t *__restrict__ M, const float *lut,
                                         int ip, int rows, int cols, int x, int y, uint32_t m) {
    const size_t p = (size_t)y * ip + x;
    const bool vl = x > 0, vr = x + 1 < cols, vu = y > 0, vd = y + 1 < rows;
    const uint32_t ml = M[p - 1], mu = M[p - ip];
    return mean4<CONTRACT>(X[p - 1], X[p + 1], X[p - ip], X[p + ip],
                           lut[ml & 255], lut[m & 255], lut[(mu >> 8) & 255], lut[(m >> 8) & 255], vl, vr, vu, vd);
}

template <bool CONTRACT>
__global__ __launch_bounds__(256) void k_residual(const float *__restrict__ X, const uint32_t *__restrict__ M,
                                                  const float *__restrict__ lut_g, int ip, int rows, int cols,
                                                  unsigned int *__restrict__ out_bits) {
    __shared__ float lut[257];
    __shared__ float wmax[4];
    for (int i = threadIdx.x; i < 257; i += 256) lut[i] = lut_g[i];
    __syncthreads();
    const int x0 = 4 * (blockIdx.x * 64 + (threadIdx.x & 63));
    const int y = blockIdx.y * 4 + wave_id();
    float d = 0.0f;
    if (x0 < cols && y < rows) {
        const size_t p = (size_t)y * ip + x0;
        const float4 c4 = *(const float4 *)(X + p), u4 = *(const float4 *)(X + p - ip), d4 = *(const float4 *)(X + p + ip);
        const uint4 m4 = *(const uint4 *)(M + p), mu4 = *(const uint4 *)(M + p - ip);
        const float xc[4] = {c4.x, c4.y, c4.z, c4.w}, xu[4] = {u4.x, u4.y, u4.z, u4.w}, xd[4] = {d4.x, d4.y, d4.z, d4.w};
        const uint32_t mm[4] = {m4.x, m4.y, m4.z, m4.w}, mu[4] = {mu4.x, mu4.y, mu4.z, mu4.w};
        const float xl0 = X[p - 1], xr4 = X[p + 4];
        const uint32_t ml0 = M[p - 1];
        const bool vu = y > 0, vd = y + 1 < rows;
#pragma unroll
        for (int i = 0; i < 4; i++) {
            const int x = x0 + i;
            if (x < cols && !(mm[i] & kMetaDirichlet)) {
                const float r = mean4<CONTRACT>(i == 0 ? xl0 : xc[i - 1], i == 3 ? xr4 : xc[i + 1], xu[i], xd[i],
                                                lut[(i == 0 ? ml0 : mm[i - 1]) & 255], lut[mm[i] & 255], lut[(mu[i] >> 8) & 255], lut[(mm[i] >> 8) & 255],
                                                x > 0, x + 1 < cols, vu, vd);
                float e = fabsf(r - xc[i]);
                if (!(e >= 0.0f)) e = __builtin_inff();
                d = fmaxf(d, e);
            }
        }
    }
#pragma unroll
    for (int s = 32; s > 0; s >>= 1) d = fmaxf(d, __shfl_xor(d, s));
    if ((threadIdx.x & 63) == 0) wmax[threadIdx.x >> 6] = d;
    __syncthreads();
    if (threadIdx.x == 0) {
        d = fmaxf(fmaxf(wmax[0], wmax[1]), fmaxf(wmax[2], wmax[3]));
        const unsigned int bits = __float_as_uint(d);
        if (bits > __hip_atomic_load(out_bits, __ATOMIC_RELAXED, __HIP_MEMORY_SCOPE_AGENT)) atomicMax(out_bits, bits);
    }
}

template <bool CONTRACT>
__global__ __launch_bounds__(256) void k_rbgs_half(float *__restrict__ X, const uint32_t *__restrict__ M,
                                                   const float *__restrict__ lut_g, int ip, int rows, int cols, int colour, float omega) {
    __shared__ float lut[257];
    for (int i = threadIdx.x; i < 257; i += 256) lut[i] = lut_g[i];
    __syncthreads();
    const int y = blockIdx.y * 4 + wave_id();
    const int x = 2 * (blockIdx.x * 64 + (threadIdx.x & 63)) + ((y + colour) & 1);
    if (x >= cols || y >= rows) return;
    const uint32_t m = M[(size_t)y * ip + x];
    if (m & kMetaDirichlet) return;
    float v = mean_at<CONTRACT>(X, M, lut, ip, rows, cols, x, y, m);
    if (omega != 1.0f) {
        const float x0 = X[(size_t)y * ip + x];
        v = CONTRACT ? __builtin_fmaf(omega, v - x0, x0) : x0 + omega * (v - x0);
        v = fminf(fmaxf(v, 0.0f), 255.0f);
    }
    X[(size_t)y * ip + x] = v;
}

static inline dim3 grid64x4(int rows, int cols, int images = 1) { return dim3((cols + 63) / 64, (rows + 3) / 4, images); }

int launch_prepare(rtdd_ctx *ctx, const Level &L, size_t ip, const SolveCall &c) {
    const Batch &B = c.targets.batch;
    const int gated = c.level != ctx->maxLevel;
    const int thr = c.level == 0 ? 0 : 4;
    const size_t zP = L.elems * sizeof(float);
    bool aligned = ((uintptr_t)c.depth % 16 == 0) && c.depthPitch % 16 == 0 && ((uintptr_t)c.gray % 4 == 0) && c.grayPitch % 4 == 0 &&
                         ((uintptr_t)c.scribble % 4 == 0) && c.scribblePitch % 4 == 0 && B.depth % 16 == 0 && B.gray % 4 == 0 && B.scribble % 4 == 0;
    const bool regions = c.regionFlags != 0;
    if (regions) aligned = aligned && ((uintptr_t)c.regions % 4 == 0) && c.regionsPitch % 4 == 0 && B.regions % 4 == 0;
    const dim3 grid = aligned ? grid64x4(c.rows, (c.cols + 3) / 4, B.n) : grid64x4(c.rows, c.cols, B.n);
    if (regions) {
        auto *kernel = c.guide == RTDD_GUIDE_BGR ? (aligned ? k_prepare4_bgr_regions : k_prepare_bgr_regions) : (aligned ? k_prepare4_regions : k_prepare_regions);
        hipLaunchKernelGGL(kernel, grid, dim3(256), 0, ctx->stream, c.depth, c.depthPitch, c.scribble, c.scribblePitch,
                           c.gray, c.grayPitch, L.P(0, ip), L.P(1, ip), L.M(ip), (int)ip, c.rows, c.cols, gated, thr, B.depth, B.scribble, B.gray, zP, ctx->sync_words, ctx->wild_seq,
                           c.regions, c.regionsPitch, B.regions, c.regionFlags);
        RTDD_LAUNCH_CHECK(ctx, "k_prepare_regions");
        return RTDD_OK;
    }
    auto *kernel = c.guide == RTDD_GUIDE_BGR ? (aligned ? k_prepare4_bgr : k_prepare_bgr) : (aligned ? k_prepare4 : k_prepare);
    hipLaunchKernelGGL(kernel, grid, dim3(256), 0, ctx->stream, c.depth, c.depthPitch, c.scribble, c.scribblePitch,
                       c.gray, c.grayPitch, L.P(0, ip), L.P(1, ip), L.M(ip), (int)ip, c.rows, c.cols, gated, thr, B.depth, B.scribble, B.gray, zP, ctx->sync_words, ctx->wild_seq);
    RTDD_LAUNCH_CHECK(ctx, "k_prepare");
    return RTDD_OK;
}

int launch_index_to_weight(rtdd_ctx *ctx, const uint8_t *gray, size_t grayPitch, const float *depth, size_t depthPitch,
                           int32_t *index2, int level, int rows, int cols, int guide, const uint8_t *regions, size_t regionsPitch, int regionFlags) {
    const int gated = level != ctx->maxLevel;
    const int thr = level == 0 ? 0 : 4;
    if (regionFlags != 0) {
        hipLaunchKernelGGL(guide == RTDD_GUIDE_BGR ? k_index_to_weight_bgr<true> : k_index_to_weight<true>, grid64x4(rows, cols), dim3(256), 0, ctx->stream,
                           gray, grayPitch, depth, depthPitch, index2, rows, cols, gated, thr, RegionImage<true>{regions, regionsPitch, regionFlags});
        RTDD_LAUNCH_CHECK(ctx, "k_index_to_weight<regions>");
        return RTDD_OK;
    }
    hipLaunchKernelGGL(guide == RTDD_GUIDE_BGR ? k_index_to_weight_bgr<false> : k_index_to_weight<false>, grid64x4(rows, cols), dim3(256), 0, ctx->stream, gray, grayPitch,
                       depth, depthPitch, index2, rows, cols, gated, thr, RegionImage<false>{});
    RTDD_LAUNCH_CHECK(ctx, "k_index_to_weight");
    return RTDD_OK;
}

static int pick_rows_per_wave(const rtdd_ctx *ctx, int rows, int cols) {
    if (ctx->opt.rows_per_wave > 0) return ctx->opt.rows_per_wave;
    const long strips = (cols + 255) / 256;
    const long want_waves = (long)ctx->num_cus * 16;
    long R = (strips * rows + want_waves - 1) / want_waves;
    if (R < 2) R = 2;
    if (R > 16) R = 16;
    return (int)R;
}

int launch_sweeps(rtdd_ctx *ctx, const Level &L, size_t ip, int rows, int cols, const float *omegas, int n,
                  int *pk, int *pm, int *launches) {
    const float gamma = 0.99;
    const int R = pick_rows_per_wave(ctx, rows, cols);
    ctx->last_info.kernel = 1; ctx->last_info.tile = 0; ctx->last_info.temporal_depth = 1; ctx->last_info.persistent = 0;
    const dim3 grid((cols + 255) / 256, (rows + 4 * R - 1) / (4 * R));
    int a = *pk, b = *pm;
    for (int it = 0; it < n; it++) {
        if (ctx->opt.fp_contract)
            hipLaunchKernelGGL(k_sweep1<true>, grid, dim3(256), 0, ctx->stream, L.P(a, ip), L.P(b, ip), L.M(ip), ctx->lut_dev,
                               (int)ip, rows, cols, R, omegas[it], gamma);
        else
            hipLaunchKernelGGL(k_sweep1<false>, grid, dim3(256), 0, ctx->stream, L.P(a, ip), L.P(b, ip), L.M(ip), ctx->lut_dev,
                               (int)ip, rows, cols, R, omegas[it], gamma);
        const int t = a; a = b; b = t;
    }
    RTDD_LAUNCH_CHECK(ctx, "k_sweep1");
    *pk = a; *pm = b;
    *launches = n;
    return RTDD_OK;
}

int launch_finish(rtdd_ctx *ctx, const Level &L, size_t ip, int src_plane, const SolveCall &c, int seq) {
    const SolveTargets &t = c.targets;
    const Batch &B = t.batch;
    const size_t zP = L.elems * sizeof(float);
    if ((uintptr_t)c.depth % 16 == 0 && c.depthPitch % 16 == 0 && B.depth % 16 == 0 && B.u8 % 4 == 0)
        hipLaunchKernelGGL(k_finish4, grid64x4(c.rows, (c.cols + 3) / 4, B.n), dim3(256), 0, ctx->stream, L.P(src_plane, ip), (int)ip, c.depth, c.depthPitch,
                           c.rows, c.cols, t.u8, t.u8_pitch, ctx->sync_words, seq, zP, B.depth, B.u8, t.u8b, t.u8b_pitch);
    else
        hipLaunchKernelGGL(k_finish, grid64x4(c.rows, c.cols, B.n), dim3(256), 0, ctx->stream, L.P(src_plane, ip), (int)ip, c.depth, c.depthPitch,
                           c.rows, c.cols, t.u8, t.u8_pitch, ctx->sync_words, seq, zP, B.depth, B.u8, t.u8b, t.u8b_pitch);
    note_publisher(ctx, seq);
    RTDD_LAUNCH_CHECK(ctx, "k_finish");
    return RTDD_OK;
}

int launch_residual(rtdd_ctx *ctx, const Level &L, size_t ip, int plane, int rows, int cols, float *host_out) {
    RTDD_HIP(ctx, hipMemsetAsync(ctx->residual_dev, 0, sizeof(float), ctx->stream));
    if (ctx->opt.fp_contract)
        hipLaunchKernelGGL(k_residual<true>, dim3((cols + 255) / 256, (rows + 3) / 4), dim3(256), 0, ctx->stream, L.P(plane, ip), L.M(ip), ctx->lut_dev,
                           (int)ip, rows, cols, (unsigned int *)ctx->residual_dev);
    else
        hipLaunchKernelGGL(k_residual<false>, dim3((cols + 255) / 256, (rows + 3) / 4), dim3(256), 0, ctx->stream, L.P(plane, ip), L.M(ip), ctx->lut_dev,
                           (int)ip, rows, cols, (unsigned int *)ctx->residual_dev);
    RTDD_LAUNCH_CHECK(ctx, "k_residual");
    RTDD_HIP(ctx, hipMemcpyAsync(host_out, ctx->residual_dev, sizeof(float), hipMemcpyDeviceToHost, ctx->stream));
    RTDD_HIP(ctx, hipStreamSynchronize(ctx->stream));
    return check_persistent_status(ctx, true);
}

int launch_rbgs(rtdd_ctx *ctx, const Level &L, size_t ip, int plane, int rows, int cols, int nsweeps, float omega) {
    ctx->last_info.kernel = 3; ctx->last_info.tile = 0; ctx->last_info.temporal_depth = 1; ctx->last_info.persistent = 0;
    const dim3 grid(((cols + 1) / 2 + 63) / 64, (rows + 3) / 4);
    for (int s = 0; s < nsweeps; s++)
        for (int colour = 0; colour < 2; colour++) {
            if (ctx->opt.fp_contract)
                hipLaunchKernelGGL(k_rbgs_half<true>, grid, dim3(256), 0, ctx->stream, L.P(plane, ip), L.M(ip), ctx->lut_dev, (int)ip, rows, cols, colour, omega);
            else
                hipLaunchKernelGGL(k_rbgs_half<false>, grid, dim3(256), 0, ctx->stream, L.P(plane, ip), L.M(ip), ctx->lut_dev, (int)ip, rows, cols, colour, omega);
        }
    RTDD_LAUNCH_CHECK(ctx, "k_rbgs_half");
    return RTDD_OK;
}

}
```

realtimedepthdiffusion_amd/csrc/sweep_blocked.hip:

```cpp
#include <type_traits>

#include "rtdd_internal.hpp"
#include "persist_sync.hpp"
#include "sweep_common.hpp"
#include "sweep_diag.hpp"

namespace rtdd {


template <bool CONTRACT, bool FAST>
__device__ __forceinline__ float relax(float xl, float xr, float xu, float xd, float wl, float wr, float wu, float wd,
                                       float cnt, float rcp, float x, float prev, float omega, float gamma) {
    float sum = 0.0f;
    sum = CONTRACT ? __builtin_fmaf(wl, xl, sum) : sum + wl * xl;
    sum = CONTRACT ? __builtin_fmaf(wr, xr, sum) : sum + wr * xr;
    sum = CONTRACT ? __builtin_fmaf(wu, xu, sum) : sum + wu * xu;
    sum = CONTRACT ? __builtin_fmaf(wd, xd, sum) : sum + wd * xd;
    float r;
    if (FAST) {
        r = div_tail(sum, cnt, rcp);
        const bool tiny = __builtin_fabsf(sum) < 0x1p-100f && sum != 0.0f;
        if (__builtin_expect(__builtin_amdgcn_ballot_w64(tiny) != 0, 0)) r = tiny ? sum / cnt : r;
    } else {
        r = sum / cnt;
    }
    r = __builtin_amdgcn_fmed3f(r, 0.0f, 255.0f);
    if (CONTRACT) return __builtin_fmaf(omega, __builtin_fmaf(gamma, r - x, x) - prev, prev);
    return (omega * (gamma * (r - x) + x - prev)) + prev;
}

template <int LX, int NT, int G, bool CONTRACT, bool PERSIST>
__global__ __launch_bounds__(NT, (NT >= 1024 || G <= 3 ? 4 : G <= 4 ? 3 : 2)) void k_sweep_blocked(float *Xk, float *Xm, float *Yk, float *Ym,
                                                      const uint32_t *__restrict__ M, const float *__restrict__ lut_g,
                                                      const float *__restrict__ omegas, int ip, int rows, int cols,
                                                      int hx, int hy, int nsweeps, float gamma,
                                                      int block_sweeps, int *sync_words, int gx, int gy, int xcd_tiles, int flag_base, size_t zPlane, int wild_seq, int withhold) {
    constexpr int EW = 4 * LX, NTR = NT / LX;
    __shared__ float lut[257];
    __shared__ float4 edge[2][NTR][2][LX];
    __shared__ int published[NT / 64 + 1];
    __shared__ int dead_s;
    __shared__ int4 xrec[PERSIST ? NT : 1];

    int bx = blockIdx.x, by = blockIdx.y;
    if (xcd_tiles > 0) {
        const int t = ((int)blockIdx.x & 7) * xcd_tiles + ((int)blockIdx.x >> 3);
        if (t >= gx * gy) return;
        bx = t % gx; by = t / gx;
    }
    RTDD_Z(Xk, zPlane); RTDD_Z(Xm, zPlane); RTDD_Z(Yk, zPlane); RTDD_Z(Ym, zPlane); RTDD_Z(M, zPlane);
    RTDD_STAMP(0);
    __builtin_amdgcn_s_setprio(2);
    const int tid = threadIdx.x;
    const int lx = tid % LX, tr = tid / LX;
    const int ntr = (int)blockDim.x / LX;
    const int eh = ntr * G;
    const int TW = EW - 2 * hx, TH = eh - 2 * hy;
    const int x0 = bx * TW - hx + 4 * lx;
    const int y0 = by * TH - hy + tr * G;
    const bool colok = x0 >= 0 && x0 < cols;

    typedef float f4r __attribute__((ext_vector_type(4)));
    f4r a[G], b[G];
    float wr[G][4], wd[G][4], wl0[G], wu0[4], cnt[G][4], rcp[G][4];
    bool unsafe = false;
    uint32_t dirichlet = 0;

    const int wild_word = load_wild_word(sync_words);
    float4 vxr[G], vpr[G];
    uint4 mr[G], mup = make_uint4(0, 0, 0, 0);
#pragma unroll
    for (int g = 0; g < G; g++) {
        const int y = y0 + g;
        vxr[g] = make_float4(0, 0, 0, 0); vpr[g] = vxr[g]; mr[g] = make_uint4(0, 0, 0, 0);
        if (colok && y >= 0 && y < rows) {
            const size_t off = (size_t)y * ip + x0;
            vxr[g] = *(const float4 *)(Xk + off);
            vpr[g] = *(const float4 *)(Xm + off);
            mr[g] = *(const uint4 *)(M + off);
        }
    }
    if (colok && y0 - 1 >= 0 && y0 < rows) mup = *(const uint4 *)(M + (size_t)(y0 - 1) * ip + x0);
    for (int i = tid; i < 257; i += (int)blockDim.x) lut[i] = lut_g[i];
    if (tid <= NT / 64) published[tid] = 0;
    if (tid == 0) { dead_s = PERSIST && __hip_atomic_load(&sync_words[kSyncStatus], __ATOMIC_RELAXED, __HIP_MEMORY_SCOPE_AGENT) != 0; }
    const int ntiles = gx * gy, tile_base = (int)blockIdx.z * ntiles, tile_id = by * gx + bx;
    if (PERSIST) {
        if (exchange_wait_at<false, true>(sync_words, &dead_s, tid, tile_id, exchange_poll_offset(tid, bx, by, gx, gy, tile_base), flag_base, withhold, tile_base)) return;
    } else {
        __syncthreads();
    }

    RTDD_STAMP_LOADED(4);
    const int tx0 = bx * TW - hx, ty0 = by * TH - hy;
    const bool tile_inside = tx0 >= 0 && tx0 + EW < cols && ty0 >= 1 && ty0 + eh < rows;
#include "sweep_tile_setup.inc"
    if constexpr (PERSIST) {
        const bool xin = colok & (4 * lx >= hx) & (4 * lx < EW - hx);
        uint32_t bits = 0;
#pragma unroll
        for (int g = 0; g < G; g++) {
            const int y = y0 + g, ty = tr * G + g;
            const bool central = xin & (ty >= hy) & (ty < eh - hy);
            const bool band = (ty < 2 * hy) | (ty >= eh - 2 * hy) | (4 * lx < 2 * hx) | (4 * lx >= EW - 2 * hx);
            const bool ok = colok & (y >= 0) & (y < rows);
            bits |= (uint32_t)(central & (y < rows) & band) << g;
            bits |= (uint32_t)(ok & !central) << (8 + g);
        }
        const int nv = min(max(cols - x0, 0), 4);
        bits |= (uint32_t)nv << 16;
        bits |= (uint32_t)(colok & (nv < 4)) << 19;
        const uint32_t off0 = ((uint32_t)y0 * (uint32_t)ip + (uint32_t)x0) * 4u;
        xrec[tid] = make_int4((int)off0, (int)bits, exchange_poll_offset(tid, bx, by, gx, gy, tile_base), 0);
    }

    RTDD_STAMP(1);
    __builtin_amdgcn_s_setprio(0);
#include "sweep_tile_sweeps.inc"
    int s = 0, blk = 0;
    bool odd = false, dead = false;
    RTDD_XT_BEGIN;
    for (;; blk++) {
        const int s_end = min(s + block_sweeps, nsweeps);
        publish(a[0], a[G - 1], s, 0);
        using P0 = std::integral_constant<int, 0>; using P1 = std::integral_constant<int, 1>;
        if constexpr (!PERSIST) {
            if (!wave_unsafe) {
                for (; s + 1 < s_end; s += 2) {
                    sweep(a, b, s, std::true_type{}, false, P0{});
                    sweep(b, a, s + 1, std::true_type{}, s + 2 >= s_end, P1{});
                }
                if (s < s_end) { sweep(a, b, s, std::true_type{}, true, P0{}); s++; odd = true; }
            } else {
                for (; s + 1 < s_end; s += 2) {
                    sweep(a, b, s, std::false_type{}, false, P0{});
                    sweep(b, a, s + 1, std::false_type{}, s + 2 >= s_end, P1{});
                }
                if (s < s_end) { sweep(a, b, s, std::false_type{}, true, P0{}); s++; odd = true; }
            }
        } else {
            const int s_fast = wave_unsafe ? s : s_end;
            for (; s + 1 < s_fast; s += 2) {
                sweep(a, b, s, std::true_type{}, false, P0{});
                sweep(b, a, s + 1, std::true_type{}, s + 2 >= s_end, P1{});
            }
            if (s < s_fast) { sweep(a, b, s, std::true_type{}, true, P0{}); s++; odd = true; }
            while (s < s_end) {
                const bool single = s + 1 >= s_end;
                sweep(a, b, s, std::false_type{}, single, P0{});
                if (single) { s++; odd = true; break; }
                sweep(b, a, s + 1, std::false_type{}, s + 2 >= s_end, P1{});
                s += 2;
            }
        }
        if (!PERSIST || s >= nsweeps) break;
        RTDD_XT(0);

        {
            const float *Ek = (blk & 1) ? Xk : Yk, *Em = (blk & 1) ? Xm : Ym;
            int tid_x = tid;
            asm volatile("" : "+v"(tid_x));
            const int4 rec = xrec[tid_x];
            const uint32_t off0 = (uint32_t)rec.x, bits = (uint32_t)rec.y, pitch = (uint32_t)ip * 4u;
            RTDD_XT(5);
#pragma unroll
            for (int g = 0; g < G; g++) {
                if (bits & (1u << g)) {
                    store_sc1_at(Ek, off0 + g * pitch, a[g]);
                    store_sc1_at(Em, off0 + g * pitch, b[g]);
                }
            }
            asm volatile("s_waitcnt vmcnt(0)" ::: "memory");
            __syncthreads();
            RTDD_XT(1);
#ifndef RTDD_EXCHANGE_ACQUIRE
#define RTDD_EXCHANGE_ACQUIRE 0
#endif
            if (exchange_wait_at<RTDD_EXCHANGE_ACQUIRE != 0>(sync_words, &dead_s, tid, tile_id, rec.z, flag_base + blk + 1, withhold, tile_base)) { dead = true; break; }
            RTDD_XT(2);
            RTDD_XT(3);
#if RTDD_EXCHANGE_ACQUIRE
#pragma unroll
            for (int g = 0; g < G; g++) {
                if (bits & (0x100u << g)) {
                    a[g] = *(const f4r *)((const char *)Ek + (off0 + g * pitch));
                    b[g] = *(const f4r *)((const char *)Em + (off0 + g * pitch));
                }
            }
#else
            {
                uint32_t off[G];
                unsigned long long lanes[G];
#pragma unroll
                for (int g = 0; g < G; g++) { off[g] = off0 + g * pitch; lanes[g] = __builtin_amdgcn_ballot_w64((bits & (0x100u << g)) != 0); }
                RTDD_XT(6);
                load_halo_rows_sc1<G>(a, b, Ek, Em, off, lanes);
                RTDD_XT(7);
            }
#endif
            if (__builtin_amdgcn_ballot_w64((bits & (1u << 19)) != 0) != 0) {
                asm volatile("");
                const int nv = (int)((bits >> 16) & 7u);
#pragma unroll
                for (int g = 0; g < G; g++) {
                    if (bits & (0x100u << g)) {
#pragma unroll
                        for (int i = 0; i < 4; i++) { const bool in = i < nv; a[g][i] = in ? a[g][i] : 0.0f; b[g][i] = in ? b[g][i] : 0.0f; }
                    }
                }
            }
        }
        (void)ntiles;
        RTDD_XT(4);
    }
    if (PERSIST && dead) return;
    if (PERSIST && (blk & 1)) { Yk = Xk; Ym = Xm; }
    RTDD_STAMP(2);

    int tid_w = tid;
    asm volatile("" : "+v"(tid_w));
    const int lx_w = tid_w % LX, tr_w = tid_w / LX;
    const int x0_w = bx * TW - hx + 4 * lx_w, y0_w = by * TH - hy + tr_w * G;
    const bool xin_w = x0_w >= 0 && x0_w < cols && 4 * lx_w >= hx && 4 * lx_w < EW - hx;
#pragma unroll
    for (int g = 0; g < G; g++) {
        const int y = y0_w + g, ty = tr_w * G + g, x0 = x0_w;
        if (xin_w && ty >= hy && ty < eh - hy && y < rows) {
            const size_t off = (size_t)y * ip + x0;
            const float4 vk = make_float4(odd ? b[g][0] : a[g][0], odd ? b[g][1] : a[g][1], odd ? b[g][2] : a[g][2], odd ? b[g][3] : a[g][3]);
            const float4 vm = make_float4(odd ? a[g][0] : b[g][0], odd ? a[g][1] : b[g][1], odd ? a[g][2] : b[g][2], odd ? a[g][3] : b[g][3]);
            store_result((float4 *)(Yk + off), vk);
            store_result((float4 *)(Ym + off), vm);
        }
    }
    RTDD_STAMP_LAST(3);
}

template <bool CONTRACT>
__global__ __launch_bounds__(1024) void k_sweep_col(const float *__restrict__ Xk, const float *__restrict__ Xm, float *__restrict__ Yk, float *__restrict__ Ym,
                                                    const uint32_t *__restrict__ M, const float *__restrict__ lut_g, const float *__restrict__ omegas,
                                                    int ip, int rows, int cols, int hx, int hy, int nsweeps, float gamma, int gx, int gy, int xcd_tiles, int *sync_words, size_t zPlane, int wild_seq) {
    constexpr int R = 4;
    RTDD_Z(Xk, zPlane); RTDD_Z(Xm, zPlane); RTDD_Z(Yk, zPlane); RTDD_Z(Ym, zPlane); RTDD_Z(M, zPlane);
    __shared__ float lut[257];
    __shared__ int4 edge[2][16][64];
    int bx = blockIdx.x, by = blockIdx.y;
    if (xcd_tiles > 0) {
        const int t = ((int)blockIdx.x & 7) * xcd_tiles + ((int)blockIdx.x >> 3);
        if (t >= gx * gy) return;
        bx = t % gx; by = t / gx;
    }
    const int tid = threadIdx.x, lane = tid & 63;
    const int wv = __builtin_amdgcn_readfirstlane(tid >> 6), nwv = (int)blockDim.x >> 6;
    const int eh = R * nwv, TW = 64 - 2 * hx, TH = eh - 2 * hy;
    const int x = bx * TW - hx + lane, y0 = by * TH - hy + R * wv;
    const bool colok = x >= 0 && x < cols;
    float a[R], b[R], wr[R], wd[R], wl[R], cnt[R], rcp[R], wu0;
    bool dir[R], unsafe = false;
    const int wild_word = load_wild_word(sync_words);
    uint32_t mraw[R], mup = 0;
#pragma unroll
    for (int g = 0; g < R; g++) {
        const int y = y0 + g;
        const bool in = colok && y >= 0 && y < rows;
        const size_t off = (size_t)(in ? y : 0) * ip + (in ? x : 0);
        mraw[g] = in ? M[off] : 0u;
        a[g] = in ? Xk[off] : 0.0f;
        b[g] = in ? Xm[off] : 0.0f;
    }
    {
        const int y = y0 - 1;
        if (colok && y >= 0 && y + 1 < rows) mup = M[(size_t)y * ip + x];
    }
    for (int i = tid; i < 257; i += (int)blockDim.x) lut[i] = lut_g[i];
    for (int i = tid; i < 2 * 16 * 64; i += (int)blockDim.x) (&edge[0][0][0])[i] = make_int4(0, 0, 0, 0);
    __syncthreads();
#pragma unroll
    for (int g = 0; g < R; g++) {
        const int y = y0 + g;
        const bool in = colok && y >= 0 && y < rows;
        const uint32_t m = mraw[g];
        wr[g] = (in && x + 1 < cols) ? lut[m & 255] : 0.0f;
        wd[g] = (in && y + 1 < rows) ? lut[(m >> 8) & 255] : 0.0f;
        dir[g] = in && (m & kMetaDirichlet);
        wl[g] = lane_from_prev(wr[g]);
    }
    {
        const int y = y0 - 1;
        const bool ok = colok && y >= 0 && y + 1 < rows;
        wu0 = ok ? lut[(mup >> 8) & 255] : 0.0f;
    }
#pragma unroll
    for (int g = 0; g < R; g++) {
        float c = 0.0f;
        c += wl[g]; c += wr[g]; c += g == 0 ? wu0 : wd[g - 1]; c += wd[g];
        cnt[g] = c == 0.0f ? 1.0f : c;
        rcp[g] = rcp_rn(cnt[g]);
        unsafe |= cnt[g] < 0x1p-126f;
    }
    const bool wave_unsafe = __builtin_amdgcn_ballot_w64(unsafe) != 0 || wild_word == wild_seq;
    constexpr uint32_t kTinyT = 2u * 0x0D800000u - 1u;
    const int up_w = wv > 0 ? wv - 1 : wv, dn_w = wv < nwv - 1 ? wv + 1 : wv;
    const int up_half = wv > 0 ? 1 : 0, dn_half = wv < nwv - 1 ? 0 : 1;
    auto publish = [&](int buf, float top, float bottom, int tag) {
        int *e = (int *)&edge[buf][wv][lane];
        asm volatile("" ::: "memory");
        e[0] = __float_as_int(top); e[2] = __float_as_int(bottom);
        asm volatile("" ::: "memory");
        __hip_atomic_store(&e[1], tag, __ATOMIC_RELAXED, __HIP_MEMORY_SCOPE_WORKGROUP);
        __hip_atomic_store(&e[3], tag, __ATOMIC_RELAXED, __HIP_MEMORY_SCOPE_WORKGROUP);
        asm volatile("" ::: "memory");
    };

    bool gone = false;
    const int tile_id_tl = by * gx + bx; (void)tile_id_tl;
    auto sweep = [&](float (&cur)[R], float (&oth)[R], int s, auto fast, bool last, auto parity) {
        constexpr bool FAST = decltype(fast)::value;
        constexpr int buf = decltype(parity)::value;
        float up, dn;
        RTDD_TL(0, s);
        {
            const long long *pu = (const long long *)&edge[buf][up_w][lane] + up_half, *pd = (const long long *)&edge[buf][dn_w][lane] + dn_half;
            auto read_both = [&]() {
                const long long u = __hip_atomic_load(pu, __ATOMIC_RELAXED, __HIP_MEMORY_SCOPE_WORKGROUP);
                const long long d = __hip_atomic_load(pd, __ATOMIC_RELAXED, __HIP_MEMORY_SCOPE_WORKGROUP);
                up = __int_as_float((int)u); dn = __int_as_float((int)d);
                const int tu = (int)(u >> 32), td = (int)(d >> 32);
                return __builtin_amdgcn_ballot_w64((tu < td ? tu : td) < s + 1) == 0;
            };
            if (__builtin_expect(!read_both(), 0)) {
                unsigned spins = 0;
                while (!gone) {
                    __builtin_amdgcn_s_sleep(1);
                    if (read_both()) break;
                    if (++spins > (1u << 22)) {
                        __hip_atomic_store(&sync_words[kSyncStatus], 2, __ATOMIC_RELAXED, __HIP_MEMORY_SCOPE_AGENT);
                        gone = true;
                    }
                }
                if (gone) { up = 0.0f; dn = 0.0f; }
            }
        }
        RTDD_TL_ROWS_IN_HAND(s);
        const float omega = omegas[s], gamma_v = gamma;
        auto wsum = [&](int g) {
            const float xl = lane_from_prev(cur[g]);
            const float xu = g == 0 ? up : cur[g - 1], xd = g == R - 1 ? dn : cur[g + 1];
            const float wu = g == 0 ? wu0 : wd[g - 1];
            float sum = 0.0f;
            sum = CONTRACT ? __builtin_fmaf(wl[g], xl, sum) : sum + wl[g] * xl;
            if (CONTRACT) {
                asm volatile("v_fmac_f32_dpp %0, %1, %2 wave_shl:1 row_mask:0xf bank_mask:0xf bound_ctrl:1" : "+v"(sum) : "v"(cur[g]), "v"(wr[g]));
            } else {
                sum = sum + wr[g] * lane_from_next(cur[g]);
            }
            sum = CONTRACT ? __builtin_fmaf(wu, xu, sum) : sum + wu * xu;
            sum = CONTRACT ? __builtin_fmaf(wd[g], xd, sum) : sum + wd[g] * xd;
            return sum;
        };
        auto pair = [&](int g0, int g1) {
            const float s0 = wsum(g0), s1 = wsum(g1);
            float q0, q1;
            if (FAST) {
                q0 = div_tail(s0, cnt[g0], rcp[g0]); q1 = div_tail(s1, cnt[g1], rcp[g1]);
                const uint32_t t0 = (__float_as_uint(s0) << 1) + 0xFFFFFFFFu, t1 = (__float_as_uint(s1) << 1) + 0xFFFFFFFFu;
                if (__builtin_expect(__builtin_amdgcn_ballot_w64((t0 < t1 ? t0 : t1) < kTinyT) != 0, 0)) {
                    q0 = div_tiny(s0, cnt[g0], rcp[g0]); q1 = div_tiny(s1, cnt[g1], rcp[g1]);
                }
            } else { q0 = s0 / cnt[g0]; q1 = s1 / cnt[g1]; }
            const int gs[2] = {g0, g1}; const float qs[2] = {q0, q1};
#pragma unroll
            for (int k = 0; k < 2; k++) {
                const int g = gs[k];
                const float r = __builtin_amdgcn_fmed3f(qs[k], 0.0f, 255.0f);
                const float xc = cur[g], prev = oth[g];
                const float v = CONTRACT ? __builtin_fmaf(omega, __builtin_fmaf(gamma_v, r - xc, xc) - prev, prev)
                                         : (omega * (gamma_v * (r - xc) + xc - prev)) + prev;
                oth[g] = dir[g] ? xc : v;
            }
        };
        __builtin_amdgcn_s_setprio(1);
        pair(0, R - 1);
        if (!last) publish(buf ^ 1, oth[0], oth[R - 1], s + 2);
        __builtin_amdgcn_s_setprio(0);
        RTDD_TL(2, s);
        pair(1, 2);
        RTDD_TL(3, s);
    };

    publish(0, a[0], a[R - 1], 1);
    using P0 = std::integral_constant<int, 0>; using P1 = std::integral_constant<int, 1>;
    const int n = nsweeps;
    const int a0 = n + 2 - hy + R * wv, a1 = n - 2 - R * wv + eh - hy;
    const int active_until = min(n - 1, min(a0, a1));
    int s = 0;
    bool odd = false;
    if (!wave_unsafe) {
        for (; s + 1 < n && s + 1 <= active_until; s += 2) { sweep(a, b, s, std::true_type{}, false, P0{}); sweep(b, a, s + 1, std::true_type{}, s + 2 >= n, P1{}); }
        if (s < n && s <= active_until) { sweep(a, b, s, std::true_type{}, s + 1 >= n, P0{}); odd = true; }
    } else {
        for (; s + 1 < n && s + 1 <= active_until; s += 2) { sweep(a, b, s, std::false_type{}, false, P0{}); sweep(b, a, s + 1, std::false_type{}, s + 2 >= n, P1{}); }
        if (s < n && s <= active_until) { sweep(a, b, s, std::false_type{}, s + 1 >= n, P0{}); odd = true; }
    }
    if (active_until < n - 1) {
        for (int bf = 0; bf < 2; bf++) {
            int *e = (int *)&edge[bf][wv][lane];
            __hip_atomic_store(&e[1], 0x7FFFFFFF, __ATOMIC_RELAXED, __HIP_MEMORY_SCOPE_WORKGROUP);
            __hip_atomic_store(&e[3], 0x7FFFFFFF, __ATOMIC_RELAXED, __HIP_MEMORY_SCOPE_WORKGROUP);
        }
        return;
    }
    const bool xin = colok && lane >= hx && lane < 64 - hx;
#pragma unroll
    for (int g = 0; g < R; g++) {
        const int y = y0 + g, ty = R * wv + g;
        if (xin && ty >= hy && ty < eh - hy && y < rows) {
            const size_t off = (size_t)y * ip + x;
            Yk[off] = odd ? b[g] : a[g];
            Ym[off] = odd ? a[g] : b[g];
        }
    }
}

struct TileCfg { int lx, nt, g; };
static const TileCfg kTiles[] = {{0, 0, 0}, {16, 256, 4}, {32, 512, 4}, {32, 1024, 4}, {32, 1024, 3}, {32, 512, 3}, {16, 512, 3}, {16, 256, 3}, {32, 1024, 2},
                                 {16, 1024, 1}, {16, 512, 2}, {32, 1024, 1}, {32, 768, 4}, {32, 512, 6},
                                 {16, 1024, 1} ,
                                 {16, 512, 1} , {16, 768, 1} };
constexpr int kNumTiles = 16;
static inline bool is_col_tile(int tile) { return tile >= 14; }
static inline int tile_rows(int tile, int nthreads) { return nthreads / kTiles[tile].lx * kTiles[tile].g; }

template <typename K>
static bool fits_one_per_cu(K kernel, int nthreads) {
    int nb = 0;
    return hipOccupancyMaxActiveBlocksPerMultiprocessor(&nb, kernel, nthreads, 0) == hipSuccess && nb >= 1;
}

template <int LX, int NT, int G>
static bool persistent_possible(rtdd_ctx *ctx, int tile, int nthreads) {
    signed char &c = ctx->persist_fit[tile][ctx->opt.fp_contract ? 1 : 0];
    if (c < 0) c = ctx->opt.fp_contract ? fits_one_per_cu(k_sweep_blocked<LX, NT, G, true, true>, nthreads) : fits_one_per_cu(k_sweep_blocked<LX, NT, G, false, true>, nthreads);
    return c == 1;
}

template <int LX, int NT, int G>
static void launch_cfg(rtdd_ctx *ctx, dim3 grid, int xcd_tiles, int nthreads, float *Xk, float *Xm, float *Yk, float *Ym, const uint32_t *M,
                       const float *omegas, int ip, int rows, int cols, int hx, int hy, int n, float gamma, int block_sweeps, int flag_base, size_t zPlane, int images) {
    const bool persist = block_sweeps < n;
    const dim3 launch_grid = xcd_tiles > 0 ? dim3(8 * xcd_tiles, 1, images) : dim3(grid.x, grid.y, images);
#define RTDD_LAUNCH(C, P) hipLaunchKernelGGL((k_sweep_blocked<LX, NT, G, C, P>), launch_grid, dim3(nthreads), 0, ctx->stream, Xk, Xm, Yk, Ym, M, ctx->lut_dev, omegas, ip, rows, cols, hx, hy, n, gamma, block_sweeps, ctx->sync_words, (int)grid.x, (int)grid.y, xcd_tiles, flag_base, zPlane, ctx->wild_seq, ctx->opt.debug_withhold_tile)
    if (ctx->opt.fp_contract) { if (persist) RTDD_LAUNCH(true, true); else RTDD_LAUNCH(true, false); }
    else { if (persist) RTDD_LAUNCH(false, true); else RTDD_LAUNCH(false, false); }
#undef RTDD_LAUNCH
}

static const int kWgPerCu[kNumTiles + 1] = {0, 3, 1, 1, 1, 2, 2, 4, 1, 2, 2, 2, 1, 1, 2, 4, 2};

static double config_cost(const rtdd_ctx *ctx, int rows, int cols, int n, int tile, int T, bool persist, int images = 1) {
    const int G = kTiles[tile].g;
    const int EW = 4 * kTiles[tile].lx, EH = tile_rows(tile, kTiles[tile].nt);
    const int hx = (T + 3) / 4 * 4, TW = EW - 2 * hx, TH = EH - 2 * T;
    if (TW < 8 || TH < 8) return 1e30;
    const double nwg = (double)((cols + TW - 1) / TW) * ((rows + TH - 1) / TH) * images;
    const double cus = ctx->num_cus, ext = (double)EW * EH;
    const double lat = 0.25 + 0.28 * G;
    const double thr1 = 1.5 * ext / 12288.0;
    const double img_bytes = (double)rows * cols * 20.0 * images;
    const double small = img_bytes < 2e6 ? 0.5 : 1.0;
    const double bw = img_bytes > 2e8 ? 17600.0 : 22600.0;
    const double load1 = small * ext * 12.0 / bw, store1 = small * (double)TW * TH * 8.0 / bw;
    if (persist) {
        if (is_col_tile(tile) || nwg > cus || (T & 1) || hx > TW || T > TH || n <= T) return 1e30;
        return (T * (lat > thr1 ? lat : thr1) + 5.0 + 3.0 * ext / 12288.0) / T;
    }
    const int k = kWgPerCu[tile];
    const double boundary = small < 1.0 ? 3.5 : 6.0;
    const double m = nwg / cus;
    double t;
    if (m <= k) {
        const double on_cu = m < 1.0 ? 1.0 : ceil(m);
        const double thr = thr1 * on_cu;
        t = boundary + load1 * on_cu + T * (lat > thr ? lat : thr) + 0.5;
    } else if (k >= 2) {
        const double rounds = ceil(nwg / (cus * k));
        const double m_eff = rounds <= 3 ? rounds * k : m;
        const double comp = (images > 1 && G >= 3 ? 0.95 : 1.45) * T * thr1, mem = load1 + store1;
        t = boundary + load1 + m_eff * (comp > mem ? comp : mem);
    } else {
        t = boundary + ceil(m) * (load1 + T * (lat > thr1 ? lat : thr1) + 0.5 * store1);
    }
    if (tile == 14) { if (m > k) return 1e30; t *= 0.9; }
    return t / T;
}

static double choose_config(const rtdd_ctx *ctx, int rows, int cols, int n, int fixed_tile, int fixed_T, int *tile, int *T, bool *persist, int images) {
    static const int tiles[] = {4, 8, 9, 14, 6, 5, 7, 12};
    static const int depths[] = {4, 8, 12, 16, 24, 28};
    double best = 1e30;
    *tile = 9; *T = 8; *persist = false;
    for (int ti : tiles) {
        if (fixed_tile && ti != fixed_tile) continue;
        for (int d : depths) {
            if (fixed_T && d != fixed_T) continue;
            for (int p = 0; p < 2; p++) {
                if (p && !ctx->opt.persistent) continue;
                const double c = config_cost(ctx, rows, cols, n, ti, d, p != 0, images);
                if (c < best) { best = c; *tile = ti; *T = d; *persist = p != 0; }
            }
        }
    }
    if (fixed_tile && best >= 1e30) *tile = fixed_tile;
    if (fixed_T && best >= 1e30) *T = fixed_T;
    return best;
}

#define RTDD_ALL_TILES \
    RTDD_TILE_CASE(1, 16, 256, 4) RTDD_TILE_CASE(2, 32, 512, 4) RTDD_TILE_CASE(3, 32, 1024, 4) RTDD_TILE_CASE(4, 32, 1024, 3) RTDD_TILE_CASE(5, 32, 512, 3) \
    RTDD_TILE_CASE(6, 16, 512, 3) RTDD_TILE_CASE(7, 16, 256, 3) RTDD_TILE_CASE(8, 32, 1024, 2) RTDD_TILE_CASE(9, 16, 1024, 1) RTDD_TILE_CASE(10, 16, 512, 2) \
    RTDD_TILE_CASE(11, 32, 1024, 1) RTDD_TILE_CASE(12, 32, 768, 4) RTDD_TILE_CASE(13, 32, 512, 6)

static int launch_sweeps_blocked_impl(rtdd_ctx *ctx, const Level &L, size_t ip, int rows, int cols, const float *omegas_dev, int n, int *pk, int *pm, int *launches, int images);

int launch_sweeps_blocked(rtdd_ctx *ctx, const Level &L, size_t ip, int rows, int cols, const float *omegas_dev, int n,
                          int *pk, int *pm, int *launches, int images) {
    if (images > 1 && ctx->opt.tile == 0 && ctx->opt.temporal_depth == 0 && !(cols <= 128 && rows <= 96)) {
        int t1, T1, tb, Tb; bool p1, pb;
        const double c1 = choose_config(ctx, rows, cols, n, 0, 0, &t1, &T1, &p1, 1);
        const double cb = choose_config(ctx, rows, cols, n, 0, 0, &tb, &Tb, &pb, images);
        if (p1 && 0.6 * c1 * images < cb) {
            int rc = RTDD_OK, a = *pk, b = *pm, total = 0;
            for (int i = 0; i < images && rc == RTDD_OK; i++) {
                a = *pk; b = *pm;
                int ln = 0;
                rc = launch_sweeps_blocked_impl(ctx, L.view(i), ip, rows, cols, omegas_dev, n, &a, &b, &ln, 1);
                total += ln;
            }
            *pk = a; *pm = b; *launches = total;
            return rc;
        }
    }
    return launch_sweeps_blocked_impl(ctx, L, ip, rows, cols, omegas_dev, n, pk, pm, launches, images);
}

static int launch_sweeps_blocked_impl(rtdd_ctx *ctx, const Level &L, size_t ip, int rows, int cols, const float *omegas_dev, int n,
                                      int *pk, int *pm, int *launches, int images) {
    const float gamma = 0.99;
    int tile = ctx->opt.tile, T = ctx->opt.temporal_depth;
    bool want_persistent = ctx->opt.persistent != 0;
    if (tile == 0 || T == 0) {
        int bt = 0, bT = 0; bool bp = false;
        if (cols <= 64 && rows <= 64) { bt = 9; bT = 8; }
        else if (cols <= 128 && rows <= 32) { bt = 11; bT = 8; }
        else if (images > 1 && cols <= 128 && rows <= 96) { bt = 4; bT = 8; }
        else choose_config(ctx, rows, cols, n, tile, T, &bt, &bT, &bp, images);
        if (tile == 0) tile = bt;
        if (T == 0) T = bT;
        if (ctx->opt.tile == 0 && ctx->opt.temporal_depth == 0) want_persistent = want_persistent && bp;
    }
    if (tile < 1 || tile > kNumTiles) tile = 1;
    const int EW = 4 * kTiles[tile].lx, EH = tile_rows(tile, kTiles[tile].nt);
    const bool single = cols <= EW && rows <= EH;
    if (T > 28) T = 28;
    while (T > 1 && (EW - 2 * ((T + 3) / 4 * 4) < 8 || EH - 2 * T < 8)) T--;
    int done = 0;
    *launches = 0;
    ctx->last_nominal_depth = single ? n : T;
    while (done < n) {
        int m = single ? n - done : (n - done < T ? n - done : T);
        const int hy = single ? 0 : (n - done < T ? n - done : T);
        const int hx = single ? 0 : (hy + 3) / 4 * 4;
        int nthreads = kTiles[tile].nt;
        if (single) {
            const int need = (rows + kTiles[tile].g - 1) / kTiles[tile].g * kTiles[tile].lx;
            nthreads = (need + 63) / 64 * 64;
            if (nthreads > kTiles[tile].nt) nthreads = kTiles[tile].nt;
        }
        const int eh = tile_rows(tile, nthreads);
        const int TW = EW - 2 * hx, TH = eh - 2 * hy;
        const dim3 grid((cols + TW - 1) / TW, (rows + TH - 1) / TH);
        int block_sweeps = m;
        bool persistent = !single && want_persistent && (int)(grid.x * grid.y) * images <= ctx->num_cus && grid.x * grid.y * images <= (unsigned)kSyncMaxTiles &&
                                (T % 2 == 0) && n - done > T && hy == T &&
                                hx <= TW && hy <= TH &&
                                (size_t)rows * ip * sizeof(float) < ((size_t)1 << 32);
        if (is_col_tile(tile)) persistent = false;
        if (persistent) {
#define RTDD_TILE_CASE(id, LX_, NT_, G_) case id: persistent = persistent_possible<LX_, NT_, G_>(ctx, tile, kTiles[tile].nt); break;
            switch (tile) { RTDD_ALL_TILES }
#undef RTDD_TILE_CASE
        }
        int flag_base = 0;
        if (persistent) {
            block_sweeps = T;
            m = n - done;
            RTDD_TRY(prepare_persistent_launch(ctx, (m + T - 1) / T, &flag_base));
            note_status_writer(ctx);
        }
        const int xcd_tiles = !single ? ((int)(grid.x * grid.y) + 7) / 8 : 0;
        int free0 = -1, free1 = -1;
        for (int i = 0; i < 4; i++) if (i != *pk && i != *pm) { if (free0 < 0) free0 = i; else free1 = i; }
        float *Xk = L.P(*pk, ip), *Xm = L.P(*pm, ip);
        float *Yk = L.P(free0, ip), *Ym = L.P(free1, ip);
        const size_t zPlane = L.elems * sizeof(float);
#define RTDD_TILE_CASE(id, LX_, NT_, G_) \
    case id: launch_cfg<LX_, NT_, G_>(ctx, grid, xcd_tiles, nthreads, Xk, Xm, Yk, Ym, L.M(ip), omegas_dev + done, (int)ip, rows, cols, hx, hy, m, gamma, block_sweeps, flag_base, zPlane, images); break;
        if (is_col_tile(tile)) {
            const dim3 launch_grid = xcd_tiles > 0 ? dim3(8 * xcd_tiles, 1, images) : dim3(grid.x, grid.y, images);
            if (ctx->opt.fp_contract) hipLaunchKernelGGL(k_sweep_col<true>, launch_grid, dim3(nthreads), 0, ctx->stream, Xk, Xm, Yk, Ym, L.M(ip), ctx->lut_dev, omegas_dev + done, (int)ip, rows, cols, hx, hy, m, gamma, (int)grid.x, (int)grid.y, xcd_tiles, ctx->sync_words, zPlane, ctx->wild_seq);
            else hipLaunchKernelGGL(k_sweep_col<false>, launch_grid, dim3(nthreads), 0, ctx->stream, Xk, Xm, Yk, Ym, L.M(ip), ctx->lut_dev, omegas_dev + done, (int)ip, rows, cols, hx, hy, m, gamma, (int)grid.x, (int)grid.y, xcd_tiles, ctx->sync_words, zPlane, ctx->wild_seq);
        } else
        switch (tile) { RTDD_ALL_TILES }
#undef RTDD_TILE_CASE
        note_status_writer(ctx);
        if (ctx->opt.debug_force_status) {
            RTDD_HIP(ctx, hipMemsetD32Async((hipDeviceptr_t)(ctx->sync_words + kSyncStatus), ctx->opt.debug_force_status == 3 ? 1 : ctx->opt.debug_force_status, 1, ctx->stream));
            ctx->opt.debug_force_status = 0;
        }
        ctx->last_info.kernel = 2; ctx->last_info.tile = tile; ctx->last_info.temporal_depth = persistent ? block_sweeps : m; ctx->last_info.persistent = persistent ? 1 : 0;
        ctx->last_launch_images = images;
        const int nblocks = (m + block_sweeps - 1) / block_sweeps;
        if (((nblocks - 1) & 1) == 0) { *pk = free0; *pm = free1; }
        done += m;
        (*launches)++;
    }
    RTDD_LAUNCH_CHECK(ctx, "k_sweep_blocked");
    return RTDD_OK;
}

}
```

realtimedepthdiffusion_amd/csrc/sweep_common.hpp:

```cpp
#pragma once
#include <hip/hip_runtime.h>

namespace rtdd {

__device__ __forceinline__ float lane_from_prev(float v) {
    return __int_as_float(__builtin_amdgcn_update_dpp(0, __float_as_int(v), 0x138, 0xF, 0xF, true));
}
__device__ __forceinline__ float lane_from_next(float v) {
    return __int_as_float(__builtin_amdgcn_update_dpp(0, __float_as_int(v), 0x130, 0xF, 0xF, true));
}

__device__ __forceinline__ float lds_from_prev(int prev4, float v) { return __int_as_float(__builtin_amdgcn_ds_bpermute(prev4, __float_as_int(v))); }
__device__ __forceinline__ float lds_from_next(int prev4, float v) { return __int_as_float(__builtin_amdgcn_ds_bpermute(prev4 + 8, __float_as_int(v))); }

typedef float f4v_t __attribute__((ext_vector_type(4)));
__device__ __forceinline__ void store_sc1_at(const float *base, uint32_t off, f4v_t v) {
    asm volatile("s_nop 4\n\tglobal_store_dwordx4 %0, %1, %2 sc1\n\ts_nop 1" ::"v"(off), "v"(v), "s"(base) : "memory");
}
#define RTDD_HALO_ROW(n) "s_and_b64 exec, %[sv], %[m" #n "]\n\tglobal_load_dwordx4 %[a" #n "], %[o" #n "], %[bk] sc1\n\tglobal_load_dwordx4 %[b" #n "], %[o" #n "], %[bm] sc1\n\t"
#define RTDD_HALO_OUT(n) [a##n] "+v"(a[n]), [b##n] "+v"(b[n])
#define RTDD_HALO_IN(n) [o##n] "v"(off[n]), [m##n] "s"(mask[n])
#define RTDD_HALO_ASM(rows, outs, ins) asm volatile("s_nop 2\n\ts_mov_b64 %[sv], exec\n\t" rows "s_mov_b64 exec, %[sv]\n\ts_waitcnt vmcnt(0)" : outs, [sv] "=&s"(sv) : ins, [bk] "s"(bk), [bm] "s"(bm) : "memory", "scc")
#define RTDD_C ,
template <int G>
__device__ __forceinline__ void load_halo_rows_sc1(f4v_t (&a)[G], f4v_t (&b)[G], const float *bk, const float *bm, const uint32_t (&off)[G], const unsigned long long (&mask)[G]) {
    unsigned long long sv;
    if constexpr (G == 1) RTDD_HALO_ASM(RTDD_HALO_ROW(0), RTDD_HALO_OUT(0), RTDD_HALO_IN(0));
    else if constexpr (G == 2) RTDD_HALO_ASM(RTDD_HALO_ROW(0) RTDD_HALO_ROW(1), RTDD_HALO_OUT(0) RTDD_C RTDD_HALO_OUT(1), RTDD_HALO_IN(0) RTDD_C RTDD_HALO_IN(1));
    else if constexpr (G == 3) RTDD_HALO_ASM(RTDD_HALO_ROW(0) RTDD_HALO_ROW(1) RTDD_HALO_ROW(2), RTDD_HALO_OUT(0) RTDD_C RTDD_HALO_OUT(1) RTDD_C RTDD_HALO_OUT(2),
                                             RTDD_HALO_IN(0) RTDD_C RTDD_HALO_IN(1) RTDD_C RTDD_HALO_IN(2));
    else if constexpr (G == 4) RTDD_HALO_ASM(RTDD_HALO_ROW(0) RTDD_HALO_ROW(1) RTDD_HALO_ROW(2) RTDD_HALO_ROW(3), RTDD_HALO_OUT(0) RTDD_C RTDD_HALO_OUT(1) RTDD_C RTDD_HALO_OUT(2) RTDD_C RTDD_HALO_OUT(3),
                                             RTDD_HALO_IN(0) RTDD_C RTDD_HALO_IN(1) RTDD_C RTDD_HALO_IN(2) RTDD_C RTDD_HALO_IN(3));
    else {
        static_assert(G == 6, "add a statement for this G");
        RTDD_HALO_ASM(RTDD_HALO_ROW(0) RTDD_HALO_ROW(1) RTDD_HALO_ROW(2) RTDD_HALO_ROW(3) RTDD_HALO_ROW(4) RTDD_HALO_ROW(5),
                      RTDD_HALO_OUT(0) RTDD_C RTDD_HALO_OUT(1) RTDD_C RTDD_HALO_OUT(2) RTDD_C RTDD_HALO_OUT(3) RTDD_C RTDD_HALO_OUT(4) RTDD_C RTDD_HALO_OUT(5),
                      RTDD_HALO_IN(0) RTDD_C RTDD_HALO_IN(1) RTDD_C RTDD_HALO_IN(2) RTDD_C RTDD_HALO_IN(3) RTDD_C RTDD_HALO_IN(4) RTDD_C RTDD_HALO_IN(5));
    }
}
#undef RTDD_C
#undef RTDD_HALO_ASM
#undef RTDD_HALO_IN
#undef RTDD_HALO_OUT
#undef RTDD_HALO_ROW

__device__ __forceinline__ void store_result(float4 *p, float4 v) { *p = v; }

__device__ __forceinline__ float div_tail(float n, float d, float y) {
    const float q0 = n * y;
    const float r = __builtin_fmaf(-d, q0, n);
    return __builtin_fmaf(r, y, q0);
}

__device__ __forceinline__ float div_tiny(float n, float d, float y) {
    const bool tiny = __builtin_fabsf(n) < 0x1p-100f;
    const float up = tiny ? 0x1p64f : 1.0f, down = tiny ? 0x1p-64f : 1.0f;
    const float N = n * up;
    const float qd = (N * y) * down;
    const float R = __builtin_fmaf(-d, qd * up, N);
    return __builtin_fmaf(R, y * down, qd);
}

__device__ __forceinline__ float rcp_rn(float d) {
    const float y0 = __builtin_amdgcn_rcpf(d);
    return __builtin_fmaf(__builtin_fmaf(-d, y0, 1.0f), y0, y0);
}

__device__ __forceinline__ void masked_fmac4(float &o0, float &o1, float &o2, float &o3, float w, float t0, float t1, float t2, float t3,
                                             unsigned long long m0, unsigned long long m1, unsigned long long m2, unsigned long long m3) {
    unsigned long long entry;
    asm("s_and_saveexec_b64 %[e], %[m0]\n\tv_fmac_f32_e32 %[o0], %[w], %[t0]\n\t"
        "s_and_b64 exec, %[e], %[m1]\n\tv_fmac_f32_e32 %[o1], %[w], %[t1]\n\t"
        "s_and_b64 exec, %[e], %[m2]\n\tv_fmac_f32_e32 %[o2], %[w], %[t2]\n\t"
        "s_and_b64 exec, %[e], %[m3]\n\tv_fmac_f32_e32 %[o3], %[w], %[t3]\n\t"
        "s_mov_b64 exec, %[e]"
        : [o0] "+v"(o0), [o1] "+v"(o1), [o2] "+v"(o2), [o3] "+v"(o3), [e] "=&s"(entry)
        : [w] "v"(w), [t0] "v"(t0), [t1] "v"(t1), [t2] "v"(t2), [t3] "v"(t3), [m0] "s"(m0), [m1] "s"(m1), [m2] "s"(m2), [m3] "s"(m3)
        : "scc");
}
__device__ __forceinline__ void masked_add4(float &o0, float &o1, float &o2, float &o3, float p0, float p1, float p2, float p3,
                                            unsigned long long m0, unsigned long long m1, unsigned long long m2, unsigned long long m3) {
    unsigned long long entry;
    asm("s_and_saveexec_b64 %[e], %[m0]\n\tv_add_f32_e32 %[o0], %[p0], %[o0]\n\t"
        "s_and_b64 exec, %[e], %[m1]\n\tv_add_f32_e32 %[o1], %[p1], %[o1]\n\t"
        "s_and_b64 exec, %[e], %[m2]\n\tv_add_f32_e32 %[o2], %[p2], %[o2]\n\t"
        "s_and_b64 exec, %[e], %[m3]\n\tv_add_f32_e32 %[o3], %[p3], %[o3]\n\t"
        "s_mov_b64 exec, %[e]"
        : [o0] "+v"(o0), [o1] "+v"(o1), [o2] "+v"(o2), [o3] "+v"(o3), [e] "=&s"(entry)
        : [p0] "v"(p0), [p1] "v"(p1), [p2] "v"(p2), [p3] "v"(p3), [m0] "s"(m0), [m1] "s"(m1), [m2] "s"(m2), [m3] "s"(m3)
        : "scc");
}

}
```

realtimedepthdiffusion_amd/csrc/sweep_tile_setup.inc:

```
    auto finish_setup = [&]() {
#pragma unroll
        for (int g = 0; g < G; g++)
#pragma unroll
            for (int i = 0; i < 4; i++) {
                const float wl = i == 0 ? wl0[g] : wr[g][i - 1];
                const float wu = g == 0 ? wu0[i] : wd[g - 1][i];
                float c = 0.0f;
                c += wl; c += wr[g][i]; c += wu; c += wd[g][i];
                cnt[g][i] = c == 0.0f ? 1.0f : c;
                rcp[g][i] = rcp_rn(cnt[g][i]);
                unsafe |= cnt[g][i] < 0x1p-126f;
            }
    };
    if (tile_inside) {
#pragma unroll
        for (int g = 0; g < G; g++) {
            const auto vx = vxr[g], vp = vpr[g];
            const uint4 m = mr[g];
            const float xv[4] = {vx.x, vx.y, vx.z, vx.w}, pv[4] = {vp.x, vp.y, vp.z, vp.w};
            const uint32_t mv[4] = {m.x, m.y, m.z, m.w};
#pragma unroll
            for (int i = 0; i < 4; i++) {
                a[g][i] = xv[i];
                b[g][i] = pv[i];
                wr[g][i] = lut[mv[i] & 255];
                wd[g][i] = lut[(mv[i] >> 8) & 255];
                dirichlet |= ((mv[i] >> 16) & 1u) << (g * 4 + i);
            }
            if (lx == LX - 1) wr[g][3] = 0.0f;
            wl0[g] = lane_from_prev(wr[g][3]);
        }
        {
            const uint32_t mv[4] = {mup.x, mup.y, mup.z, mup.w};
#pragma unroll
            for (int i = 0; i < 4; i++) wu0[i] = lut[(mv[i] >> 8) & 255];
        }
        finish_setup();
    } else {
#pragma unroll
        for (int g = 0; g < G; g++) {
            const int y = y0 + g;
            const bool ok = colok && y >= 0 && y < rows;
            const auto vx = vxr[g], vp = vpr[g];
            const uint4 m = mr[g];
            const float xv[4] = {vx.x, vx.y, vx.z, vx.w}, pv[4] = {vp.x, vp.y, vp.z, vp.w};
            const uint32_t mv[4] = {m.x, m.y, m.z, m.w};
#pragma unroll
            for (int i = 0; i < 4; i++) {
                const bool in = ok && x0 + i < cols;
                a[g][i] = in ? xv[i] : 0.0f;
                b[g][i] = in ? pv[i] : 0.0f;
                wr[g][i] = lut[(in && x0 + i + 1 < cols) ? (mv[i] & 255) : 256u];
                wd[g][i] = lut[(in && y + 1 < rows) ? ((mv[i] >> 8) & 255) : 256u];
                if (in && (mv[i] & kMetaDirichlet)) dirichlet |= 1u << (g * 4 + i);
            }
            if (lx == LX - 1) wr[g][3] = 0.0f;
            wl0[g] = lane_from_prev(wr[g][3]);
        }
        {
            const int y = y0 - 1;
            const uint4 m = mup;
            const bool ok = colok && y >= 0 && y + 1 < rows;
            const uint32_t mv[4] = {m.x, m.y, m.z, m.w};
#pragma unroll
            for (int i = 0; i < 4; i++) wu0[i] = lut[(ok && x0 + i < cols) ? ((mv[i] >> 8) & 255) : 256u];
        }
        finish_setup();
    }
    const bool wave_unsafe = __builtin_amdgcn_ballot_w64(unsafe) != 0 || wild_word == wild_seq;
    unsigned long long free_mask[G][4];
#pragma unroll
    for (int g = 0; g < G; g++)
#pragma unroll
        for (int i = 0; i < 4; i++) {
            const bool dir = (dirichlet >> (g * 4 + i)) & 1u;
            free_mask[g][i] = __builtin_amdgcn_ballot_w64(!dir);
            b[g][i] = dir ? a[g][i] : b[g][i];
        }
```

Baseline: 1.663 million.

## Use 16-bit metadata and NaN-tagged Dirichlet flags in non-persistent sweep

Adds a parallel 16-bit metadata plane holding only the right/down weight indices. Dirichlet pixels are now marked by storing a NaN tag value in the second solution plane. Non-persistent blocked sweeps read the half-width metadata and infer the Dirichlet mask from the tag instead of a 32-bit meta word, cutting per-sweep metadata bandwidth. This needs extra prepare writes, tag re-insertion on stores, a host-side state flag tracking whether Xm is tagged, and a fallback reload of the full metadata when the state is unknown or depth is wild.

Measured after the change: 1.663 million. About the same (-0.0%).

```diff
diff --git a/realtimedepthdiffusion_amd/csrc/api.cpp b/realtimedepthdiffusion_amd/csrc/api.cpp
--- a/realtimedepthdiffusion_amd/csrc/api.cpp
+++ b/realtimedepthdiffusion_amd/csrc/api.cpp
@@ -37,6 +37,7 @@
         for (auto &p : L.plane)
             if (p) { (void)hipFree(p); p = nullptr; }
         if (L.meta) { (void)hipFree(L.meta); L.meta = nullptr; }
+        if (L.meta16) { (void)hipFree(L.meta16); L.meta16 = nullptr; }
     }
     ctx->levels.clear();
     ctx->maxLevel = -1;
@@ -245,8 +246,12 @@
         hipError_t e = hipMalloc((void **)&L.meta, all * sizeof(uint32_t));
         if (e != hipSuccess) { free_levels(ctx); return fail(ctx, e == hipErrorOutOfMemory ? RTDD_ERR_NOMEM : RTDD_ERR_HIP,
             "hipMalloc(meta)", e); }
+        e = hipMalloc((void **)&L.meta16, all * sizeof(uint16_t));
+        if (e != hipSuccess) { free_levels(ctx); return fail(ctx, e == hipErrorOutOfMemory ? RTDD_ERR_NOMEM : RTDD_ERR_HIP,
+            "hipMalloc(meta16)", e); }
         for (auto &p : L.plane) RTDD_HIP(ctx, hipMemsetAsync(p, 0, all * sizeof(float), ctx->stream));
         RTDD_HIP(ctx, hipMemsetAsync(L.meta, 0, all * sizeof(uint32_t), ctx->stream));
+        RTDD_HIP(ctx, hipMemsetAsync(L.meta16, 0, all * sizeof(uint16_t), ctx->stream));
     }
     ctx->levels_images = images;
     ctx->maxLevel = levels - 1;
diff --git a/realtimedepthdiffusion_amd/csrc/rtdd_internal.hpp b/realtimedepthdiffusion_amd/csrc/rtdd_internal.hpp
--- a/realtimedepthdiffusion_amd/csrc/rtdd_internal.hpp
+++ b/realtimedepthdiffusion_amd/csrc/rtdd_internal.hpp
@@ -20,18 +20,22 @@
 inline size_t plane_elems(int rows, int cols) { return plane_pitch(cols) * (size_t)(rows + 2 * kGuardRows) + 1024; }
 
 constexpr uint32_t kMetaDirichlet = 1u << 16;
+constexpr uint32_t kDirichletTag = 0x7FA5C3E1u;
 
 struct Level {
     int rows = 0, cols = 0;
     size_t elems = 0;
     float *plane[4] = {nullptr, nullptr, nullptr, nullptr};
     uint32_t *meta = nullptr;
+    uint16_t *meta16 = nullptr;
     float *P(int i, size_t ip) const { return plane[i] + (size_t)kGuardRows * ip; }
     uint32_t *M(size_t ip) const { return meta + (size_t)kGuardRows * ip; }
+    uint16_t *M16(size_t ip) const { return meta16 + (size_t)kGuardRows * ip; }
     Level view(int b) const {
         Level v = *this;
         for (auto &q : v.plane) if (q) q += (size_t)b * elems;
         if (v.meta) v.meta += (size_t)b * elems;
+        if (v.meta16) v.meta16 += (size_t)b * elems;
         return v;
     }
 };
@@ -209,6 +213,7 @@
     bool defocus_table_sticky = false;
     int flag_epoch = 0;
     int sync_limit = 0;
+    bool xm_tagged = false;
     int last_nominal_depth = 0;
     int last_launch_images = 1;
     rtdd_solve_info last_info{};
diff --git a/realtimedepthdiffusion_amd/csrc/solver_kernels.hip b/realtimedepthdiffusion_amd/csrc/solver_kernels.hip
--- a/realtimedepthdiffusion_amd/csrc/solver_kernels.hip
+++ b/realtimedepthdiffusion_amd/csrc/solver_kernels.hip
@@ -19,19 +19,43 @@
 #define RTDD_PREPARE_PARAMS(g, gp, zg)                                                                                                      \
     const float *__restrict__ depth, size_t depthPitch, const uint8_t *__restrict__ scribble, size_t scribblePitch,                         \
     const uint8_t *__restrict__ g, size_t gp, float *__restrict__ X0, float *__restrict__ X1, uint32_t *__restrict__ M, int ip, int rows,    \
-    int cols, int gated, int thr, size_t zDepth, size_t zScribble, size_t zg, size_t zPlane, int *sync_words, int wild_seq
+    int cols, int gated, int thr, size_t zDepth, size_t zScribble, size_t zg, size_t zPlane, int *sync_words, int wild_seq, uint16_t *__restrict__ M16
 #define RTDD_PREPARE_ARGS(g, gp, zg) \
-    depth, depthPitch, scribble, scribblePitch, g, gp, X0, X1, M, ip, rows, cols, gated, thr, zDepth, zScribble, zg, zPlane, sync_words, wild_seq
+    depth, depthPitch, scribble, scribblePitch, g, gp, X0, X1, M, ip, rows, cols, gated, thr, zDepth, zScribble, zg, zPlane, sync_words, wild_seq, M16
 #define RTDD_REGION_PARAMS const uint8_t *__restrict__ codes, size_t codesPitch, size_t zCodes, int regionFlags
 #define RTDD_REGION_ARGS codes, codesPitch, zCodes, regionFlags
 #define RTDD_NO_REGIONS nullptr, 0, 0, 0
 
+__device__ __forceinline__ void store_prepared(float *X0, float *X1, uint32_t *M, uint16_t *M16, size_t p, float d, bool dirichlet, int right, int down) {
+    const uint32_t idx = (uint32_t)right | ((uint32_t)down << 8);
+    X0[p] = d;
+    X1[p] = dirichlet ? __uint_as_float(kDirichletTag) : 0.0f;
+    M[p] = idx | (dirichlet ? kMetaDirichlet : 0u);
+    M16[p] = (uint16_t)idx;
+}
+__device__ __forceinline__ void store_prepared4(float *X0, float *X1, uint32_t *M, uint16_t *M16, size_t p, const float (&d)[5], uint32_t scribble4,
+                                                const int (&right)[4], const int (&down)[4]) {
+    float x1v[4];
+    uint32_t mv[4], idx[4];
+#pragma unroll
+    for (int i = 0; i < 4; i++) {
+        const bool dirichlet = ((scribble4 >> (8 * i)) & 255) == 255;
+        idx[i] = (uint32_t)right[i] | ((uint32_t)down[i] << 8);
+        x1v[i] = dirichlet ? __uint_as_float(kDirichletTag) : 0.0f;
+        mv[i] = idx[i] | (dirichlet ? kMetaDirichlet : 0u);
+    }
+    *(float4 *)(X0 + p) = make_float4(d[0], d[1], d[2], d[3]);
+    *(float4 *)(X1 + p) = make_float4(x1v[0], x1v[1], x1v[2], x1v[3]);
+    *(uint4 *)(M + p) = make_uint4(mv[0], mv[1], mv[2], mv[3]);
+    *(uint2 *)(M16 + p) = make_uint2(idx[0] | (idx[1] << 16), idx[2] | (idx[3] << 16));
+}
+
 template <bool REGIONS>
 __device__ __forceinline__ void prepare_px(RTDD_PREPARE_PARAMS(gray, grayPitch, zGray), RTDD_REGION_PARAMS) {
     const int x = blockIdx.x * 64 + (threadIdx.x & 63);
     const int y = blockIdx.y * 4 + wave_id();
     if (x >= cols || y >= rows) return;
-    RTDD_Z(depth, zDepth); RTDD_Z(scribble, zScribble); RTDD_Z(gray, zGray); RTDD_Z(X0, zPlane); RTDD_Z(X1, zPlane); RTDD_Z(M, zPlane);
+    RTDD_Z(depth, zDepth); RTDD_Z(scribble, zScribble); RTDD_Z(gray, zGray); RTDD_Z(X0, zPlane); RTDD_Z(X1, zPlane); RTDD_Z(M, zPlane); RTDD_Z(M16, zPlane / 2);
     const float *drow = (const float *)((const char *)depth + (size_t)y * depthPitch);
     const uint8_t *grow = gray + (size_t)y * grayPitch;
     const float d = drow[x];
@@ -55,9 +79,7 @@
     }
     const size_t p = (size_t)y * ip + x;
     if (depth_is_wild(d)) sync_words[kSyncWild] = wild_seq;
-    X0[p] = d;
-    X1[p] = dirichlet ? d : 0.0f;
-    M[p] = (uint32_t)right | ((uint32_t)down << 8) | (dirichlet ? kMetaDirichlet : 0u);
+    store_prepared(X0, X1, M, M16, p, d, dirichlet, right, down);
 }
 __global__ __launch_bounds__(256) void k_prepare(RTDD_PREPARE_PARAMS(gray, grayPitch, zGray)) {
     prepare_px<false>(RTDD_PREPARE_ARGS(gray, grayPitch, zGray), RTDD_NO_REGIONS);
@@ -93,7 +115,7 @@
     const int x0 = 4 * (blockIdx.x * 64 + (threadIdx.x & 63));
     const int y = blockIdx.y * 4 + wave_id();
     if (x0 >= cols || y >= rows) return;
-    RTDD_Z(depth, zDepth); RTDD_Z(scribble, zScribble); RTDD_Z(gray, zGray); RTDD_Z(X0, zPlane); RTDD_Z(X1, zPlane); RTDD_Z(M, zPlane);
+    RTDD_Z(depth, zDepth); RTDD_Z(scribble, zScribble); RTDD_Z(gray, zGray); RTDD_Z(X0, zPlane); RTDD_Z(X1, zPlane); RTDD_Z(M, zPlane); RTDD_Z(M16, zPlane / 2);
     const float *drow = (const float *)((const char *)depth + (size_t)y * depthPitch);
     const uint8_t *grow = gray + (size_t)y * grayPitch, *srow = scribble + (size_t)y * scribblePitch;
     const bool down_ok = y + 1 < rows;
@@ -126,31 +148,23 @@
     }
     const bool right_ok = x0 + 4 < cols;
     d[4] = right_ok ? drow[x0 + 4] : 0.0f; g[4] = right_ok ? grow[x0 + 4] : 0;
-    float x0v[4], x1v[4];
-    uint32_t mv[4];
+    int right[4], down[4];
 #pragma unroll
     for (int i = 0; i < 4; i++) {
-        const bool dirichlet = ((sc >> (8 * i)) & 255) == 255;
-        int right = 0, down = 0;
+        right[i] = 0; down[i] = 0;
         if (x0 + i + 1 < cols) {
-            right = iabs(g[i] - g[i + 1]);
-            if (gated && !(iabs(sat_u8_dev(d[i]) - sat_u8_dev(d[i + 1])) > thr)) right = 0;
-            if (REGIONS) right = region_index(right, rg.rc[i], rg.rc[i + 1], regionFlags);
+            right[i] = iabs(g[i] - g[i + 1]);
+            if (gated && !(iabs(sat_u8_dev(d[i]) - sat_u8_dev(d[i + 1])) > thr)) right[i] = 0;
+            if (REGIONS) right[i] = region_index(right[i], rg.rc[i], rg.rc[i + 1], regionFlags);
         }
         if (down_ok) {
-            down = iabs(g[i] - gd[i]);
-            if (gated && !(iabs(sat_u8_dev(d[i]) - sat_u8_dev(dd[i])) > thr)) down = 0;
-            if (REGIONS) down = region_index(down, rg.rc[i], rg.rd[i], regionFlags);
-        }
-        x0v[i] = d[i];
-        x1v[i] = dirichlet ? d[i] : 0.0f;
-        mv[i] = (uint32_t)right | ((uint32_t)down << 8) | (dirichlet ? kMetaDirichlet : 0u);
+            down[i] = iabs(g[i] - gd[i]);
+            if (gated && !(iabs(sat_u8_dev(d[i]) - sat_u8_dev(dd[i])) > thr)) down[i] = 0;
+            if (REGIONS) down[i] = region_index(down[i], rg.rc[i], rg.rd[i], regionFlags);
+        }
     }
     if (depth_is_wild(d[0]) || depth_is_wild(d[1]) || depth_is_wild(d[2]) || depth_is_wild(d[3])) sync_words[kSyncWild] = wild_seq;
-    const size_t p = (size_t)y * ip + x0;
-    *(float4 *)(X0 + p) = make_float4(x0v[0], x0v[1], x0v[2], x0v[3]);
-    *(float4 *)(X1 + p) = make_float4(x1v[0], x1v[1], x1v[2], x1v[3]);
-    *(uint4 *)(M + p) = make_uint4(mv[0], mv[1], mv[2], mv[3]);
+    store_prepared4(X0, X1, M, M16, (size_t)y * ip + x0, d, sc, right, down);
 }
 __global__ __launch_bounds__(256) void k_prepare4(RTDD_PREPARE_PARAMS(gray, grayPitch, zGray)) {
     prepare4_px<false>(RTDD_PREPARE_ARGS(gray, grayPitch, zGray), RTDD_NO_REGIONS);
@@ -206,7 +220,7 @@
     const int x = blockIdx.x * 64 + (threadIdx.x & 63);
     const int y = blockIdx.y * 4 + wave_id();
     if (x >= cols || y >= rows) return;
-    RTDD_Z(depth, zDepth); RTDD_Z(scribble, zScribble); RTDD_Z(bgr, zBgr); RTDD_Z(X0, zPlane); RTDD_Z(X1, zPlane); RTDD_Z(M, zPlane);
+    RTDD_Z(depth, zDepth); RTDD_Z(scribble, zScribble); RTDD_Z(bgr, zBgr); RTDD_Z(X0, zPlane); RTDD_Z(X1, zPlane); RTDD_Z(M, zPlane); RTDD_Z(M16, zPlane / 2);
     const float *drow = (const float *)((const char *)depth + (size_t)y * depthPitch);
     const uint8_t *crow = bgr + (size_t)y * bgrPitch + 3 * (size_t)x;
     const float d = drow[x];
@@ -230,9 +244,7 @@
     }
     const size_t p = (size_t)y * ip + x;
     if (depth_is_wild(d)) sync_words[kSyncWild] = wild_seq;
-    X0[p] = d;
-    X1[p] = dirichlet ? d : 0.0f;
-    M[p] = (uint32_t)right | ((uint32_t)down << 8) | (dirichlet ? kMetaDirichlet : 0u);
+    store_prepared(X0, X1, M, M16, p, d, dirichlet, right, down);
 }
 __global__ __launch_bounds__(256) void k_prepare_bgr(RTDD_PREPARE_PARAMS(bgr, bgrPitch, zBgr)) {
     prepare_bgr_px<false>(RTDD_PREPARE_ARGS(bgr, bgrPitch, zBgr), RTDD_NO_REGIONS);
@@ -253,7 +265,7 @@
     const int x0 = 4 * (blockIdx.x * 64 + (threadIdx.x & 63));
     const int y = blockIdx.y * 4 + wave_id();
     if (x0 >= cols || y >= rows) return;
-    RTDD_Z(depth, zDepth); RTDD_Z(scribble, zScribble); RTDD_Z(bgr, zBgr); RTDD_Z(X0, zPlane); RTDD_Z(X1, zPlane); RTDD_Z(M, zPlane);
+    RTDD_Z(depth, zDepth); RTDD_Z(scribble, zScribble); RTDD_Z(bgr, zBgr); RTDD_Z(X0, zPlane); RTDD_Z(X1, zPlane); RTDD_Z(M, zPlane); RTDD_Z(M16, zPlane / 2);
     const float *drow = (const float *)((const char *)depth + (size_t)y * depthPitch);
     const uint8_t *crow = bgr + (size_t)y * bgrPitch + 3 * (size_t)x0, *srow = scribble + (size_t)y * scribblePitch;
     const bool down_ok = y + 1 < rows;
@@ -285,31 +297,23 @@
     const bool right_ok = x0 + 4 < cols;
     d[4] = right_ok ? drow[x0 + 4] : 0.0f;
     c[4] = right_ok ? (int)*(const uint16_t *)(crow + 12) | ((int)crow[14] << 16) : 0;
-    float x0v[4], x1v[4];
-    uint32_t mv[4];
+    int right[4], down[4];
 #pragma unroll
     for (int i = 0; i < 4; i++) {
-        const bool dirichlet = ((sc >> (8 * i)) & 255) == 255;
-        int right = 0, down = 0;
+        right[i] = 0; down[i] = 0;
         if (x0 + i + 1 < cols) {
-            right = bgr_index(c[i], c[i + 1]);
-            if (gated && !(iabs(sat_u8_dev(d[i]) - sat_u8_dev(d[i + 1])) > thr)) right = 0;
-            if (REGIONS) right = region_index(right, rg.rc[i], rg.rc[i + 1], regionFlags);
+            right[i] = bgr_index(c[i], c[i + 1]);
+            if (gated && !(iabs(sat_u8_dev(d[i]) - sat_u8_dev(d[i + 1])) > thr)) right[i] = 0;
+            if (REGIONS) right[i] = region_index(right[i], rg.rc[i], rg.rc[i + 1], regionFlags);
         }
         if (down_ok) {
-            down = bgr_index(c[i], cd[i]);
-            if (gated && !(iabs(sat_u8_dev(d[i]) - sat_u8_dev(dd[i])) > thr)) down = 0;
-            if (REGIONS) down = region_index(down, rg.rc[i], rg.rd[i], regionFlags);
-        }
-        x0v[i] = d[i];
-        x1v[i] = dirichlet ? d[i] : 0.0f;
-        mv[i] = (uint32_t)right | ((uint32_t)down << 8) | (dirichlet ? kMetaDirichlet : 0u);
+            down[i] = bgr_index(c[i], cd[i]);
+            if (gated && !(iabs(sat_u8_dev(d[i]) - sat_u8_dev(dd[i])) > thr)) down[i] = 0;
+            if (REGIONS) down[i] = region_index(down[i], rg.rc[i], rg.rd[i], regionFlags);
+        }
     }
     if (depth_is_wild(d[0]) || depth_is_wild(d[1]) || depth_is_wild(d[2]) || depth_is_wild(d[3])) sync_words[kSyncWild] = wild_seq;
-    const size_t p = (size_t)y * ip + x0;
-    *(float4 *)(X0 + p) = make_float4(x0v[0], x0v[1], x0v[2], x0v[3]);
-    *(float4 *)(X1 + p) = make_float4(x1v[0], x1v[1], x1v[2], x1v[3]);
-    *(uint4 *)(M + p) = make_uint4(mv[0], mv[1], mv[2], mv[3]);
+    store_prepared4(X0, X1, M, M16, (size_t)y * ip + x0, d, sc, right, down);
 }
 __global__ __launch_bounds__(256) void k_prepare4_bgr(RTDD_PREPARE_PARAMS(bgr, bgrPitch, zBgr)) {
     prepare4_bgr_px<false>(RTDD_PREPARE_ARGS(bgr, bgrPitch, zBgr), RTDD_NO_REGIONS);
@@ -565,19 +569,20 @@
     bool aligned = ((uintptr_t)c.depth % 16 == 0) && c.depthPitch % 16 == 0 && ((uintptr_t)c.gray % 4 == 0) && c.grayPitch % 4 == 0 &&
                          ((uintptr_t)c.scribble % 4 == 0) && c.scribblePitch % 4 == 0 && B.depth % 16 == 0 && B.gray % 4 == 0 && B.scribble % 4 == 0;
     const bool regions = c.regionFlags != 0;
+    ctx->xm_tagged = true;
     if (regions) aligned = aligned && ((uintptr_t)c.regions % 4 == 0) && c.regionsPitch % 4 == 0 && B.regions % 4 == 0;
     const dim3 grid = aligned ? grid64x4(c.rows, (c.cols + 3) / 4, B.n) : grid64x4(c.rows, c.cols, B.n);
     if (regions) {
         auto *kernel = c.guide == RTDD_GUIDE_BGR ? (aligned ? k_prepare4_bgr_regions : k_prepare_bgr_regions) : (aligned ? k_prepare4_regions : k_prepare_regions);
         hipLaunchKernelGGL(kernel, grid, dim3(256), 0, ctx->stream, c.depth, c.depthPitch, c.scribble, c.scribblePitch,
-                           c.gray, c.grayPitch, L.P(0, ip), L.P(1, ip), L.M(ip), (int)ip, c.rows, c.cols, gated, thr, B.depth, B.scribble, B.gray, zP, ctx->sync_words, ctx->wild_seq,
+                           c.gray, c.grayPitch, L.P(0, ip), L.P(1, ip), L.M(ip), (int)ip, c.rows, c.cols, gated, thr, B.depth, B.scribble, B.gray, zP, ctx->sync_words, ctx->wild_seq, L.M16(ip),
                            c.regions, c.regionsPitch, B.regions, c.regionFlags);
         RTDD_LAUNCH_CHECK(ctx, "k_prepare_regions");
         return RTDD_OK;
     }
     auto *kernel = c.guide == RTDD_GUIDE_BGR ? (aligned ? k_prepare4_bgr : k_prepare_bgr) : (aligned ? k_prepare4 : k_prepare);
     hipLaunchKernelGGL(kernel, grid, dim3(256), 0, ctx->stream, c.depth, c.depthPitch, c.scribble, c.scribblePitch,
-                       c.gray, c.grayPitch, L.P(0, ip), L.P(1, ip), L.M(ip), (int)ip, c.rows, c.cols, gated, thr, B.depth, B.scribble, B.gray, zP, ctx->sync_words, ctx->wild_seq);
+                       c.gray, c.grayPitch, L.P(0, ip), L.P(1, ip), L.M(ip), (int)ip, c.rows, c.cols, gated, thr, B.depth, B.scribble, B.gray, zP, ctx->sync_words, ctx->wild_seq, L.M16(ip));
     RTDD_LAUNCH_CHECK(ctx, "k_prepare");
     return RTDD_OK;
 }
@@ -626,6 +631,7 @@
     }
     RTDD_LAUNCH_CHECK(ctx, "k_sweep1");
     *pk = a; *pm = b;
+    if (n > 0) ctx->xm_tagged = false;
     *launches = n;
     return RTDD_OK;
 }
diff --git a/realtimedepthdiffusion_amd/csrc/sweep_blocked.hip b/realtimedepthdiffusion_amd/csrc/sweep_blocked.hip
--- a/realtimedepthdiffusion_amd/csrc/sweep_blocked.hip
+++ b/realtimedepthdiffusion_amd/csrc/sweep_blocked.hip
@@ -34,7 +34,8 @@
                                                       const uint32_t *__restrict__ M, const float *__restrict__ lut_g,
                                                       const float *__restrict__ omegas, int ip, int rows, int cols,
                                                       int hx, int hy, int nsweeps, float gamma,
-                                                      int block_sweeps, int *sync_words, int gx, int gy, int xcd_tiles, int flag_base, size_t zPlane, int wild_seq, int withhold) {
+                                                      int block_sweeps, int *sync_words, int gx, int gy, int xcd_tiles, int flag_base, size_t zPlane, int wild_seq, int withhold,
+                                                      const uint16_t *__restrict__ M16, int dir32) {
     constexpr int EW = 4 * LX, NTR = NT / LX;
     __shared__ float lut[257];
     __shared__ float4 edge[2][NTR][2][LX];
@@ -49,6 +50,7 @@
         bx = t % gx; by = t / gx;
     }
     RTDD_Z(Xk, zPlane); RTDD_Z(Xm, zPlane); RTDD_Z(Yk, zPlane); RTDD_Z(Ym, zPlane); RTDD_Z(M, zPlane);
+    if constexpr (!PERSIST) RTDD_Z(M16, zPlane / 2);
     RTDD_STAMP(0);
     __builtin_amdgcn_s_setprio(2);
     const int tid = threadIdx.x;
@@ -77,10 +79,14 @@
             const size_t off = (size_t)y * ip + x0;
             vxr[g] = *(const float4 *)(Xk + off);
             vpr[g] = *(const float4 *)(Xm + off);
-            mr[g] = *(const uint4 *)(M + off);
-        }
-    }
-    if (colok && y0 - 1 >= 0 && y0 < rows) mup = *(const uint4 *)(M + (size_t)(y0 - 1) * ip + x0);
+            if constexpr (PERSIST) mr[g] = *(const uint4 *)(M + off);
+            else { const uint2 h = *(const uint2 *)(M16 + off); mr[g].x = h.x; mr[g].y = h.y; }
+        }
+    }
+    if (colok && y0 - 1 >= 0 && y0 < rows) {
+        if constexpr (PERSIST) mup = *(const uint4 *)(M + (size_t)(y0 - 1) * ip + x0);
+        else { const uint2 h = *(const uint2 *)(M16 + (size_t)(y0 - 1) * ip + x0); mup.x = h.x; mup.y = h.y; }
+    }
     for (int i = tid; i < 257; i += (int)blockDim.x) lut[i] = lut_g[i];
     if (tid <= NT / 64) published[tid] = 0;
     if (tid == 0) { dead_s = PERSIST && __hip_atomic_load(&sync_words[kSyncStatus], __ATOMIC_RELAXED, __HIP_MEMORY_SCOPE_AGENT) != 0; }
@@ -228,7 +234,12 @@
         if (xin_w && ty >= hy && ty < eh - hy && y < rows) {
             const size_t off = (size_t)y * ip + x0;
             const float4 vk = make_float4(odd ? b[g][0] : a[g][0], odd ? b[g][1] : a[g][1], odd ? b[g][2] : a[g][2], odd ? b[g][3] : a[g][3]);
-            const float4 vm = make_float4(odd ? a[g][0] : b[g][0], odd ? a[g][1] : b[g][1], odd ? a[g][2] : b[g][2], odd ? a[g][3] : b[g][3]);
+            float4 vm = make_float4(odd ? a[g][0] : b[g][0], odd ? a[g][1] : b[g][1], odd ? a[g][2] : b[g][2], odd ? a[g][3] : b[g][3]);
+            if constexpr (!PERSIST) {
+                const float tag = __uint_as_float(kDirichletTag);
+                vm.x = select_free(free_mask[g][0], vm.x, tag); vm.y = select_free(free_mask[g][1], vm.y, tag);
+                vm.z = select_free(free_mask[g][2], vm.z, tag); vm.w = select_free(free_mask[g][3], vm.w, tag);
+            }
             store_result((float4 *)(Yk + off), vk);
             store_result((float4 *)(Ym + off), vm);
         }
@@ -445,11 +456,13 @@
 }
 
 template <int LX, int NT, int G>
-static void launch_cfg(rtdd_ctx *ctx, dim3 grid, int xcd_tiles, int nthreads, float *Xk, float *Xm, float *Yk, float *Ym, const uint32_t *M,
+static void launch_cfg(rtdd_ctx *ctx, dim3 grid, int xcd_tiles, int nthreads, float *Xk, float *Xm, float *Yk, float *Ym, const uint32_t *M, const uint16_t *M16,
                        const float *omegas, int ip, int rows, int cols, int hx, int hy, int n, float gamma, int block_sweeps, int flag_base, size_t zPlane, int images) {
     const bool persist = block_sweeps < n;
+    const int dir32 = !persist && !ctx->xm_tagged;
+    ctx->xm_tagged = !persist;
     const dim3 launch_grid = xcd_tiles > 0 ? dim3(8 * xcd_tiles, 1, images) : dim3(grid.x, grid.y, images);
-#define RTDD_LAUNCH(C, P) hipLaunchKernelGGL((k_sweep_blocked<LX, NT, G, C, P>), launch_grid, dim3(nthreads), 0, ctx->stream, Xk, Xm, Yk, Ym, M, ctx->lut_dev, omegas, ip, rows, cols, hx, hy, n, gamma, block_sweeps, ctx->sync_words, (int)grid.x, (int)grid.y, xcd_tiles, flag_base, zPlane, ctx->wild_seq, ctx->opt.debug_withhold_tile)
+#define RTDD_LAUNCH(C, P) hipLaunchKernelGGL((k_sweep_blocked<LX, NT, G, C, P>), launch_grid, dim3(nthreads), 0, ctx->stream, Xk, Xm, Yk, Ym, M, ctx->lut_dev, omegas, ip, rows, cols, hx, hy, n, gamma, block_sweeps, ctx->sync_words, (int)grid.x, (int)grid.y, xcd_tiles, flag_base, zPlane, ctx->wild_seq, ctx->opt.debug_withhold_tile, M16, dir32)
     if (ctx->opt.fp_contract) { if (persist) RTDD_LAUNCH(true, true); else RTDD_LAUNCH(true, false); }
     else { if (persist) RTDD_LAUNCH(false, true); else RTDD_LAUNCH(false, false); }
 #undef RTDD_LAUNCH
@@ -604,8 +617,9 @@
         float *Yk = L.P(free0, ip), *Ym = L.P(free1, ip);
         const size_t zPlane = L.elems * sizeof(float);
 #define RTDD_TILE_CASE(id, LX_, NT_, G_) \
-    case id: launch_cfg<LX_, NT_, G_>(ctx, grid, xcd_tiles, nthreads, Xk, Xm, Yk, Ym, L.M(ip), omegas_dev + done, (int)ip, rows, cols, hx, hy, m, gamma, block_sweeps, flag_base, zPlane, images); break;
+    case id: launch_cfg<LX_, NT_, G_>(ctx, grid, xcd_tiles, nthreads, Xk, Xm, Yk, Ym, L.M(ip), L.M16(ip), omegas_dev + done, (int)ip, rows, cols, hx, hy, m, gamma, block_sweeps, flag_base, zPlane, images); break;
         if (is_col_tile(tile)) {
+            ctx->xm_tagged = false;
             const dim3 launch_grid = xcd_tiles > 0 ? dim3(8 * xcd_tiles, 1, images) : dim3(grid.x, grid.y, images);
             if (ctx->opt.fp_contract) hipLaunchKernelGGL(k_sweep_col<true>, launch_grid, dim3(nthreads), 0, ctx->stream, Xk, Xm, Yk, Ym, L.M(ip), ctx->lut_dev, omegas_dev + done, (int)ip, rows, cols, hx, hy, m, gamma, (int)grid.x, (int)grid.y, xcd_tiles, ctx->sync_words, zPlane, ctx->wild_seq);
             else hipLaunchKernelGGL(k_sweep_col<false>, launch_grid, dim3(nthreads), 0, ctx->stream, Xk, Xm, Yk, Ym, L.M(ip), ctx->lut_dev, omegas_dev + done, (int)ip, rows, cols, hx, hy, m, gamma, (int)grid.x, (int)grid.y, xcd_tiles, ctx->sync_words, zPlane, ctx->wild_seq);
diff --git a/realtimedepthdiffusion_amd/csrc/sweep_common.hpp b/realtimedepthdiffusion_amd/csrc/sweep_common.hpp
--- a/realtimedepthdiffusion_amd/csrc/sweep_common.hpp
+++ b/realtimedepthdiffusion_amd/csrc/sweep_common.hpp
@@ -43,6 +43,12 @@
 #undef RTDD_HALO_IN
 #undef RTDD_HALO_OUT
 #undef RTDD_HALO_ROW
+
+__device__ __forceinline__ float select_free(unsigned long long mask, float if_set, float if_clear) {
+    float r;
+    asm("v_cndmask_b32_e64 %0, %1, %2, %3" : "=v"(r) : "v"(if_clear), "v"(if_set), "s"(mask));
+    return r;
+}
 
 __device__ __forceinline__ void store_result(float4 *p, float4 v) { *p = v; }
 
diff --git a/realtimedepthdiffusion_amd/csrc/sweep_tile_setup.inc b/realtimedepthdiffusion_amd/csrc/sweep_tile_setup.inc
--- a/realtimedepthdiffusion_amd/csrc/sweep_tile_setup.inc
+++ b/realtimedepthdiffusion_amd/csrc/sweep_tile_setup.inc
@@ -1,3 +1,11 @@
+    auto meta_px = [](const uint4 &m, int i) -> uint32_t {
+        if constexpr (PERSIST) return i == 0 ? m.x : i == 1 ? m.y : i == 2 ? m.z : m.w;
+        else { const uint32_t h = i < 2 ? m.x : m.y; return (i & 1) ? h >> 16 : h & 0xFFFFu; }
+    };
+    auto dirichlet_px = [](uint32_t mv, float prev) -> bool {
+        if constexpr (PERSIST) return (mv & kMetaDirichlet) != 0;
+        else return __float_as_uint(prev) == kDirichletTag;
+    };
     auto finish_setup = [&]() {
 #pragma unroll
         for (int g = 0; g < G; g++)
@@ -18,20 +26,20 @@
             const auto vx = vxr[g], vp = vpr[g];
             const uint4 m = mr[g];
             const float xv[4] = {vx.x, vx.y, vx.z, vx.w}, pv[4] = {vp.x, vp.y, vp.z, vp.w};
-            const uint32_t mv[4] = {m.x, m.y, m.z, m.w};
+            const uint32_t mv[4] = {meta_px(m, 0), meta_px(m, 1), meta_px(m, 2), meta_px(m, 3)};
 #pragma unroll
             for (int i = 0; i < 4; i++) {
                 a[g][i] = xv[i];
                 b[g][i] = pv[i];
                 wr[g][i] = lut[mv[i] & 255];
                 wd[g][i] = lut[(mv[i] >> 8) & 255];
-                dirichlet |= ((mv[i] >> 16) & 1u) << (g * 4 + i);
+                dirichlet |= (uint32_t)dirichlet_px(mv[i], pv[i]) << (g * 4 + i);
             }
             if (lx == LX - 1) wr[g][3] = 0.0f;
             wl0[g] = lane_from_prev(wr[g][3]);
         }
         {
-            const uint32_t mv[4] = {mup.x, mup.y, mup.z, mup.w};
+            const uint32_t mv[4] = {meta_px(mup, 0), meta_px(mup, 1), meta_px(mup, 2), meta_px(mup, 3)};
 #pragma unroll
             for (int i = 0; i < 4; i++) wu0[i] = lut[(mv[i] >> 8) & 255];
         }
@@ -44,7 +52,7 @@
             const auto vx = vxr[g], vp = vpr[g];
             const uint4 m = mr[g];
             const float xv[4] = {vx.x, vx.y, vx.z, vx.w}, pv[4] = {vp.x, vp.y, vp.z, vp.w};
-            const uint32_t mv[4] = {m.x, m.y, m.z, m.w};
+            const uint32_t mv[4] = {meta_px(m, 0), meta_px(m, 1), meta_px(m, 2), meta_px(m, 3)};
 #pragma unroll
             for (int i = 0; i < 4; i++) {
                 const bool in = ok && x0 + i < cols;
@@ -52,7 +60,7 @@
                 b[g][i] = in ? pv[i] : 0.0f;
                 wr[g][i] = lut[(in && x0 + i + 1 < cols) ? (mv[i] & 255) : 256u];
                 wd[g][i] = lut[(in && y + 1 < rows) ? ((mv[i] >> 8) & 255) : 256u];
-                if (in && (mv[i] & kMetaDirichlet)) dirichlet |= 1u << (g * 4 + i);
+                if (in && dirichlet_px(mv[i], pv[i])) dirichlet |= 1u << (g * 4 + i);
             }
             if (lx == LX - 1) wr[g][3] = 0.0f;
             wl0[g] = lane_from_prev(wr[g][3]);
@@ -61,13 +69,29 @@
             const int y = y0 - 1;
             const uint4 m = mup;
             const bool ok = colok && y >= 0 && y + 1 < rows;
-            const uint32_t mv[4] = {m.x, m.y, m.z, m.w};
+            const uint32_t mv[4] = {meta_px(m, 0), meta_px(m, 1), meta_px(m, 2), meta_px(m, 3)};
 #pragma unroll
             for (int i = 0; i < 4; i++) wu0[i] = lut[(ok && x0 + i < cols) ? ((mv[i] >> 8) & 255) : 256u];
         }
         finish_setup();
     }
-    const bool wave_unsafe = __builtin_amdgcn_ballot_w64(unsafe) != 0 || wild_word == wild_seq;
+    const bool wild = wild_word == wild_seq;
+    const bool wave_unsafe = __builtin_amdgcn_ballot_w64(unsafe) != 0 || wild;
+    if constexpr (!PERSIST) {
+        if (wild || dir32) {
+            dirichlet = 0;
+#pragma unroll
+            for (int g = 0; g < G; g++) {
+                const int y = y0 + g;
+                if (colok && y >= 0 && y < rows) {
+                    const uint4 m = *(const uint4 *)(M + (size_t)y * ip + x0);
+                    const uint32_t mv[4] = {m.x, m.y, m.z, m.w};
+#pragma unroll
+                    for (int i = 0; i < 4; i++) if (x0 + i < cols && (mv[i] & kMetaDirichlet)) dirichlet |= 1u << (g * 4 + i);
+                }
+            }
+        }
+    }
     unsigned long long free_mask[G][4];
 #pragma unroll
     for (int g = 0; g < G; g++)
```
